# Zhiyu014/GNN-UDS

Hardware: AMD Instinct MI355X
Metric: graph-steps/sec (forward rollout), |V|=10k |E|=12k d=64 (higher is better)
Workload: dtype f32 storage/accumulate, GEMM operands as bf16 hi+lo split (3 MFMA products)

## Files before the change

### gnn_uds_amd/_lib.py

```python
import ctypes
import os

import numpy as np
import torch

_HERE = os.path.dirname(os.path.abspath(__file__))
LIB_PATH = os.environ.get('UDS_LIB_PATH') or os.path.join(_HERE, 'libuds_hip.so')

ABI_VERSION = 22
FLAG_EXACT_FP32, FLAG_REQUIRE_FUSED = 1, 2
PRECISION_FLAGS = {'bf16x3': 0, 'fp32': FLAG_EXACT_FP32}

ACT = {None: 0, 'linear': 0, 'relu': 1, 'tanh': 2, 'sigmoid': 3, 'hard_sigmoid': 4}

_c_i64 = ctypes.c_int64
_c_int = ctypes.c_int
_c_ptr = ctypes.c_void_p

SYMBOLS = {
    'uds_abi_version': (_c_int, []),
    'uds_last_error': (ctypes.c_char_p, []),
    'uds_csr_create': (_c_int, [_c_ptr, _c_ptr, _c_i64, _c_i64, _c_i64, ctypes.POINTER(_c_ptr)]),
    'uds_csr_destroy': (_c_int, [_c_ptr]),
    'uds_csr_shape': (_c_int, [_c_ptr, ctypes.POINTER(_c_i64), ctypes.POINTER(_c_i64), ctypes.POINTER(_c_i64),
                               ctypes.POINTER(ctypes.c_int32)]),
    'uds_csr_row_order': (_c_int, [_c_ptr, _c_ptr]),
    'uds_dense_act': (_c_int, [_c_ptr, _c_i64, _c_ptr, _c_i64, _c_i64, _c_ptr, _c_ptr, _c_i64, _c_int, _c_ptr, _c_ptr,
                               _c_ptr, _c_ptr, _c_ptr, _c_ptr]),
    'uds_csr_spmm': (_c_int, [_c_ptr, _c_ptr, _c_ptr, _c_i64, _c_i64, _c_ptr, _c_int, _c_ptr, _c_ptr]),
    'uds_conv1d_causal': (_c_int, [_c_ptr, _c_i64, _c_i64, _c_i64, _c_i64, _c_ptr, _c_ptr, _c_i64, _c_i64, _c_i64, _c_int, _c_ptr,
                                   _c_ptr]),
    'uds_dense_cumsum_heads': (_c_int, [_c_ptr, _c_i64, _c_i64, _c_i64, _c_ptr, _c_ptr, _c_ptr, _c_int, _c_ptr, _c_ptr, _c_ptr]),
    'uds_recurrent_fused': (_c_int, [_c_ptr, _c_i64, _c_ptr, _c_ptr, _c_ptr, _c_i64, _c_i64, _c_i64, _c_int, _c_ptr, _c_ptr]),
    'uds_recurrent_fused_supported': (_c_int, [_c_i64, _c_int]),
    'uds_recurrent_forward': (_c_int, [_c_ptr, _c_ptr, _c_ptr, _c_i64, _c_i64, _c_i64, _c_i64, _c_int, _c_ptr, _c_ptr]),
    'uds_attn_sum_pool': (_c_int, [_c_ptr, _c_ptr, _c_i64, _c_i64, _c_i64, _c_ptr, _c_ptr]),
    'uds_dropout': (_c_int, [_c_ptr, _c_i64, ctypes.c_float, ctypes.c_uint64, ctypes.c_uint64, _c_ptr, _c_ptr]),
    'uds_recurrent_forward_train': (_c_int, [_c_ptr, _c_ptr, _c_ptr, _c_i64, _c_i64, _c_i64, _c_i64, _c_int, _c_ptr, _c_ptr, _c_ptr]),
    'uds_recurrent_backward': (_c_int, [_c_ptr, _c_ptr, _c_ptr, _c_ptr, _c_ptr, _c_ptr, _c_i64, _c_i64, _c_i64, _c_int, _c_ptr, _c_ptr, _c_ptr]),
    'uds_recurrent_bwd_packed_bytes': (_c_i64, [_c_i64, _c_int]),
    'uds_recurrent_pack_bwd': (_c_int, [_c_ptr, _c_i64, _c_int, _c_ptr, _c_ptr]),
    'uds_recurrent_backward_h': (_c_int, [_c_ptr, _c_ptr, _c_ptr, _c_ptr, _c_ptr, _c_ptr, _c_i64, _c_i64, _c_i64, _c_i64, _c_int, _c_ptr, _c_ptr,
                                          _c_ptr]),
    'uds_rowgemm_packed_bytes': (_c_i64, [_c_i64, _c_i64]),
    'uds_rowgemm_pack': (_c_int, [_c_ptr, _c_i64, _c_i64, _c_ptr, _c_ptr]),
    'uds_gat_aggregate_masked': (_c_int, [_c_ptr, _c_ptr, _c_ptr, _c_ptr, _c_ptr, _c_ptr, _c_i64, _c_i64, _c_int, _c_ptr, _c_ptr]),
    'uds_gat_aggregate_coef': (_c_int, [_c_ptr, _c_ptr, _c_ptr, _c_ptr, _c_ptr, _c_ptr, _c_i64, _c_i64, _c_int, _c_ptr, _c_ptr]),
    'uds_diffusion_forward': (_c_int, [_c_ptr, _c_ptr, _c_ptr, _c_ptr, _c_ptr, _c_i64, _c_i64, _c_int, _c_ptr, _c_ptr]),
    'uds_diffusion_backward_workspace_floats': (_c_i64, [_c_i64, _c_i64, _c_i64, _c_i64]),
    'uds_diffusion_backward': (_c_int, [_c_ptr, _c_ptr, _c_ptr, _c_ptr, _c_ptr, _c_ptr, _c_ptr, _c_ptr, _c_ptr, _c_ptr, _c_i64, _c_i64,
                                        _c_i64, _c_int, _c_ptr, _c_ptr, _c_ptr, _c_ptr]),
    'uds_halo_pack': (_c_int, [_c_ptr, _c_i64, _c_ptr, _c_i64, _c_i64, _c_i64, _c_ptr, _c_i64, _c_ptr, _c_i64, _c_ptr, _c_ptr]),
    'uds_halo_unpack': (_c_int, [_c_ptr, _c_i64, _c_i64, _c_ptr, _c_i64, _c_ptr, _c_i64, _c_ptr, _c_i64, _c_ptr, _c_i64, _c_ptr]),
    'uds_halo_pack_all': (_c_int, [_c_ptr, _c_i64, _c_ptr, _c_i64, _c_i64, _c_i64, _c_ptr, _c_i64, _c_ptr, _c_i64, _c_ptr, _c_ptr, _c_i64,
                                   _c_ptr, _c_ptr]),
    'uds_halo_unpack_all': (_c_int, [_c_ptr, _c_i64, _c_i64, _c_ptr, _c_i64, _c_ptr, _c_i64, _c_ptr, _c_ptr, _c_i64, _c_ptr, _c_i64, _c_ptr,
                                     _c_i64, _c_ptr]),
    'uds_halo_pack_clear_all': (_c_int, [_c_ptr, _c_i64, _c_ptr, _c_i64, _c_i64, _c_i64, _c_ptr, _c_i64, _c_ptr, _c_i64, _c_ptr, _c_ptr,
                                         _c_i64, _c_ptr, _c_ptr]),
    'uds_halo_accumulate_all': (_c_int, [_c_ptr, _c_i64, _c_i64, _c_ptr, _c_ptr, _c_i64, _c_ptr, _c_i64, _c_ptr, _c_i64, _c_ptr, _c_ptr,
                                         _c_i64, _c_ptr, _c_i64, _c_ptr, _c_i64, _c_ptr]),
    'uds_remainder_packed_bytes': (_c_i64, [_c_i64, _c_i64]),
    'uds_remainder_pack': (_c_int, [_c_ptr, _c_i64, _c_i64, _c_ptr, _c_ptr]),
    'uds_remainder_workspace_bytes': (_c_i64, [_c_i64, _c_i64, _c_i64, _c_i64]),
    'uds_remainder_forward_dense': (_c_int, [_c_ptr, _c_i64, _c_i64, _c_ptr, _c_i64, _c_ptr, _c_ptr, _c_int, _c_i64, _c_i64, _c_ptr, _c_ptr, _c_ptr]),
    'uds_remainder_forward': (_c_int, [_c_ptr, _c_i64, _c_i64, _c_ptr, _c_i64, _c_i64, _c_ptr, _c_ptr, _c_ptr]),
    'uds_rowgemm_forward': (_c_int, [_c_ptr, _c_i64, _c_i64, _c_i64, _c_i64, _c_ptr, _c_ptr, _c_i64, _c_i64, _c_i64, _c_int, _c_ptr, _c_ptr]),
    'uds_rowgemm_forward_pair': (_c_int, [_c_ptr, _c_i64, _c_ptr, _c_ptr, _c_ptr, _c_ptr, _c_i64, _c_ptr, _c_ptr, _c_ptr, _c_i64, _c_i64, _c_i64, _c_i64,
                                          _c_i64, _c_i64, _c_int, _c_ptr]),
    'uds_rowgemm_forward_cat': (_c_int, [_c_ptr, _c_i64, _c_ptr, _c_i64, _c_i64, _c_i64, _c_i64, _c_ptr, _c_ptr, _c_i64, _c_i64, _c_i64, _c_int,
                                         _c_ptr, _c_i64, _c_i64, _c_ptr]),
    'uds_dense_cumsum': (_c_int, [_c_ptr, _c_i64, _c_i64, _c_i64, _c_ptr, _c_ptr, _c_ptr, _c_int, _c_ptr, _c_ptr]),
    'uds_cumsum_act': (_c_int, [_c_ptr, _c_ptr, _c_i64, _c_i64, _c_i64, _c_i64, _c_int, _c_ptr, _c_ptr]),
    'uds_flow_balance': (_c_int, [_c_ptr, _c_ptr, _c_ptr, _c_i64, _c_ptr, _c_ptr, _c_ptr, _c_ptr, _c_ptr]),
    'uds_gat_workspace_floats': (_c_i64, [_c_i64, _c_i64, _c_i64]),
    'uds_gat_forward': (_c_int, [_c_ptr, _c_ptr, _c_i64, _c_ptr, _c_i64, _c_i64, _c_ptr, _c_ptr, _c_ptr, _c_ptr, _c_i64,
                                 _c_int, _c_ptr, _c_ptr, _c_ptr]),
    'uds_gat_aggregate': (_c_int, [_c_ptr, _c_ptr, _c_ptr, _c_ptr, _c_ptr, _c_i64, _c_i64, _c_int, _c_ptr, _c_ptr]),
    'uds_gat_backward': (_c_int, [_c_ptr, _c_ptr, _c_ptr, _c_ptr, _c_ptr, _c_ptr, _c_ptr, _c_ptr, _c_ptr, _c_i64, _c_i64, _c_ptr,
                                  _c_ptr, _c_ptr, _c_ptr, _c_ptr, _c_ptr]),
    'uds_gat_backward_coef': (_c_int, [_c_ptr, _c_ptr, _c_ptr, _c_ptr, _c_ptr, _c_ptr, _c_ptr, _c_ptr, _c_ptr, _c_ptr, _c_i64, _c_i64, _c_ptr,
                                       _c_ptr, _c_ptr, _c_ptr, _c_ptr, _c_ptr]),
    'uds_gat_aggregate_ex': (_c_int, [_c_ptr, _c_ptr, _c_ptr, _c_ptr, _c_ptr, _c_ptr, _c_ptr, _c_i64, _c_i64, _c_int, _c_ptr, _c_ptr]),
    'uds_gat_backward_ex': (_c_int, [_c_ptr, _c_ptr, _c_ptr, _c_ptr, _c_ptr, _c_ptr, _c_ptr, _c_ptr, _c_ptr, _c_ptr, _c_ptr, _c_i64, _c_i64,
                                     _c_ptr, _c_ptr, _c_ptr, _c_ptr, _c_ptr, _c_ptr]),
    'uds_csr_sddmm': (_c_int, [_c_ptr, _c_ptr, _c_ptr, _c_i64, _c_i64, _c_ptr, _c_ptr]),
    'uds_wgrad_workspace_floats': (_c_i64, [_c_i64, _c_i64, _c_i64, _c_int]),
    'uds_wgrad': (_c_int, [_c_ptr, _c_ptr, _c_i64, _c_i64, _c_i64, _c_i64, _c_i64, _c_i64, _c_int, _c_ptr, _c_ptr, _c_ptr, _c_ptr]),
    'uds_network_create': (_c_int, [_c_ptr, _c_ptr, _c_ptr, _c_ptr, ctypes.POINTER(_c_ptr)]),
    'uds_network_destroy': (_c_int, [_c_ptr]),
    'uds_network_prepare': (_c_int, [_c_ptr, _c_i64, _c_i64]),
    'uds_network_plan_info': (_c_int, [_c_ptr, _c_ptr]),
    'uds_tile_plan_create': (_c_int, [_c_ptr] * 8 + [_c_i64, _c_i64] + [ctypes.c_int32] * 4 + [ctypes.POINTER(_c_ptr)]),
    'uds_tile_plan_destroy': (_c_int, [_c_ptr]),
    'uds_tile_plan_sizes': (_c_int, [_c_ptr, ctypes.POINTER(_c_i64), ctypes.POINTER(_c_i64), _c_ptr]),
    'uds_tile_plan_copy': (_c_int, [_c_ptr, _c_ptr, _c_ptr]),
    'uds_tile_plan_blocks': (_c_int, [_c_ptr, _c_ptr, ctypes.POINTER(_c_i64)]),
    'uds_roll_update': (_c_int, [_c_ptr] * 7 + [_c_i64, _c_ptr, _c_i64, _c_ptr, _c_i64, _c_i64, _c_i64, _c_int, _c_ptr, _c_ptr, _c_ptr, _c_ptr]),
    'uds_spatial_workspace_floats': (_c_i64, [_c_ptr, _c_i64, _c_i64, _c_i64]),
    'uds_spatial_packed_bytes': (_c_i64, []),
    'uds_spatial_pack_weights': (_c_int, [_c_ptr, _c_i64, _c_i64, _c_i64, _c_i64, _c_ptr, _c_ptr]),
    'uds_spatial_layer_forward': (_c_int, [_c_ptr, _c_ptr, _c_ptr, _c_i64, _c_ptr, _c_i64, _c_i64, _c_i64, _c_i64, _c_int,
                                           _c_int, _c_ptr, _c_ptr, _c_ptr, _c_ptr]),
    'uds_spatial_layer_forward_rem': (_c_int, [_c_ptr, _c_ptr, _c_ptr, _c_i64, _c_ptr, _c_i64, _c_ptr, _c_ptr, _c_i64, _c_i64, _c_i64, _c_int, _c_int,
                                      _c_ptr, _c_ptr, _c_ptr, _c_ptr]),
    'uds_spatial_layer_forward_split': (_c_int, [_c_ptr, _c_ptr, _c_ptr, _c_i64, _c_ptr, _c_i64, _c_ptr, _c_i64, _c_ptr, _c_i64, _c_i64,
                                                 _c_i64, _c_i64, _c_int, _c_int, _c_ptr, _c_ptr, _c_ptr, _c_ptr]),
}


class SpatialParams(ctypes.Structure):
    _fields_ = [(n, _c_ptr) for n in ('xe_k', 'xe_b', 'ex_k', 'ex_b', 'ne_n_val', 'ne_e_val',
                                      'gx_k', 'gx_as', 'gx_an', 'gx_b', 'ge_k', 'ge_as', 'ge_an', 'ge_b', 'packed')]


class UdsError(RuntimeError):
    pass


_lib = None


def load():
    global _lib
    if _lib is not None:
        return _lib
    if not os.path.exists(LIB_PATH):
        raise ImportError('%s is missing: the HIP engine is not built (run `python -m gnn_uds_amd.build`); '
                          'gnn_uds_amd has no CPU fallback' % LIB_PATH)
    lib = ctypes.CDLL(LIB_PATH)
    for name, (res, args) in SYMBOLS.items():
        fn = getattr(lib, name)
        fn.restype = res
        fn.argtypes = args
    if lib.uds_abi_version() != ABI_VERSION:
        raise ImportError('libuds_hip.so ABI %d, binding expects %d' % (lib.uds_abi_version(), ABI_VERSION))
    _lib = lib
    return lib


def _check(rc, what):
    if rc != 0:
        msg = load().uds_last_error()
        raise UdsError('%s failed (%d): %s' % (what, rc, msg.decode() if msg else '?'))


def _dev(t, name, allow_none=False):
    if t is None:
        if allow_none:
            return None
        raise UdsError('%s is required' % name)
    if not isinstance(t, torch.Tensor):
        raise UdsError('%s must be a torch.Tensor, got %r' % (name, type(t)))
    if not t.is_cuda:
        raise UdsError('%s is on %s: gnn_uds_amd runs on the MI355X only and has no CPU fallback' % (name, t.device))
    if t.dtype != torch.float32:
        raise UdsError('%s must be float32, got %s' % (name, t.dtype))
    if not t.is_contiguous():
        raise UdsError('%s must be contiguous' % name)
    _same_device(t.device.index, name)
    return t.data_ptr()


def _current_device():
    if not torch.cuda.is_available():
        raise UdsError('no HIP device is visible: gnn_uds_amd runs on the MI355X only and has no CPU fallback')
    return torch.cuda.current_device()


def _same_device(index, what):
    cur = _current_device()
    if index is not None and index != cur:
        raise UdsError('%s lives on cuda:%d but the current device is cuda:%d: call torch.cuda.set_device(%d) (one process per GPU) '
                       'or wrap the call in `with torch.cuda.device(%d):`' % (what, index, cur, index, index))


def _dev_i32(t, name):
    if not isinstance(t, torch.Tensor) or not t.is_cuda or t.dtype != torch.int32 or not t.is_contiguous():
        raise UdsError('%s must be a contiguous int32 HIP tensor' % name)
    _same_device(t.device.index, name)
    return t.data_ptr()


def _stream():
    return torch.cuda.current_stream().cuda_stream


def _out(out, shape, like, name):
    if out is None:
        return torch.empty(shape, device=like.device, dtype=torch.float32)
    if tuple(out.shape) != tuple(shape) or out.device != like.device:
        raise UdsError('%s must be %r on %s, got %r on %s' % (name, tuple(shape), like.device, tuple(out.shape), out.device))
    _dev(out, name)
    return out


# ... 16 lines not shown
        if self._t is None:
            rows = np.repeat(np.arange(self.n_rows, dtype=np.int64), np.diff(self._rowptr.astype(np.int64)))
            cols = self._col.astype(np.int64)
            order = np.lexsort((rows, cols))
            t_rowptr = np.zeros(self.n_cols + 1, dtype=np.int64)
            np.add.at(t_rowptr, cols + 1, 1)
            t_rowptr = np.cumsum(t_rowptr)

            class _T:
                pass
            t = _T()
            t.n_rows, t.n_cols, t.nnz = self.n_cols, self.n_rows, self.nnz
            t.rowptr, t.col = t_rowptr.astype(np.int32), rows[order].astype(np.int32)
            self._t = (CsrHandle(t), order.astype(np.int32))
        h, perm = self._t
        if not isinstance(perm, torch.Tensor) or perm.device != torch.device(device):
            perm = torch.as_tensor(np.asarray(perm.cpu() if isinstance(perm, torch.Tensor) else perm), dtype=torch.int32,
                                   device=device)
            self._t = (h, perm)
        return h, perm

    @property
    def ptr(self):
        _same_device(self.device, 'this CSR handle')
        return self._h

    def row_order(self):
        out = np.empty(self.n_rows, dtype=np.int32)
        _check(load().uds_csr_row_order(self._h, out.ctypes.data), 'uds_csr_row_order')
        return out

    def max_degree(self):
        md = ctypes.c_int32()
        _check(load().uds_csr_shape(self._h, None, None, None, ctypes.byref(md)), 'uds_csr_shape')
        return md.value

    def __del__(self):
        h, self._h = getattr(self, '_h', None), None
        if h is not None and _lib is not None:
            _lib.uds_csr_destroy(h)


class NetworkHandle:

    def __init__(self, graph):
        lib = load()
        self.graph = graph
        self.adj = CsrHandle(graph.adj)
        self.edge_adj = CsrHandle(graph.edge_adj)
        self.inc_n = CsrHandle(graph.inc_n)
        self.inc_e = CsrHandle(graph.inc_e)
        h = _c_ptr()
        self.device = _current_device()
        _check(lib.uds_network_create(self.adj.ptr, self.edge_adj.ptr, self.inc_n.ptr, self.inc_e.ptr, ctypes.byref(h)),
               'uds_network_create')
        self._h = h
        self._prepared = {(64, 64)}

    @property
    def ptr(self):
        _same_device(self.device, 'this network handle')
        return self._h

    def prepare(self, fx, fe):
        key = (int(fx), int(fe))
        if key not in self._prepared:
            _check(load().uds_network_prepare(self.ptr, key[0], key[1]), 'uds_network_prepare')
            self._prepared.add(key)

    def plan_info(self):
        info = np.zeros(8, dtype=np.int32)
        _check(load().uds_network_plan_info(self._h, info.ctypes.data), 'uds_network_plan_info')
        keys = ('fused', 'node_tiles', 'link_tiles', 'p_cap', 'q_cap', 'meta_cap', 'lds_bytes', 't_code')
        out = dict(zip(keys, (int(v) for v in info)))
        out['t_node'], out['t_link'] = out['t_code'] // 1000, out['t_code'] % 1000
        return out

    def __del__(self):
        h, self._h = getattr(self, '_h', None), None
        if h is not None and _lib is not None:
            _lib.uds_network_destroy(h)


def tile_plan(graph, t_node=48, t_link=48, p_limit=0, q_limit=0, blocks=False):
    lib = load()
    arrs = []
    for c in (graph.adj, graph.edge_adj, graph.inc_n, graph.inc_e):
        arrs += [np.ascontiguousarray(c.rowptr, dtype=np.int32), np.ascontiguousarray(c.col, dtype=np.int32)]
    h = _c_ptr()
    _check(lib.uds_tile_plan_create(*[a.ctypes.data for a in arrs], graph.n_node, graph.n_edge, t_node, t_link,
                                    p_limit, q_limit, ctypes.byref(h)), 'uds_tile_plan_create')
    try:
        nt, pl = _c_i64(), _c_i64()
        caps = np.zeros(3, dtype=np.int32)
        _check(lib.uds_tile_plan_sizes(h, ctypes.byref(nt), ctypes.byref(pl), caps.ctypes.data), 'uds_tile_plan_sizes')
        hdr = np.zeros((nt.value, 8), dtype=np.int32)
        pool = np.zeros(pl.value, dtype=np.int32)
        _check(lib.uds_tile_plan_copy(h, hdr.ctypes.data, pool.ctypes.data), 'uds_tile_plan_copy')
        blk = None
        if blocks:
            stride = _c_i64()
            if lib.uds_tile_plan_blocks(h, None, ctypes.byref(stride)) == 0:
                blk = np.zeros((nt.value, stride.value), dtype=np.int32)
                _check(lib.uds_tile_plan_blocks(h, blk.ctypes.data, ctypes.byref(stride)), 'uds_tile_plan_blocks')
    finally:
        lib.uds_tile_plan_destroy(h)
    out = dict(p_cap=int(caps[0]), q_cap=int(caps[1]), meta_cap=int(caps[2]))
    if blocks:
        out['blocks'] = blk
    return hdr, pool, out


def dense_act(xa, kernel, bias=None, act='linear', xb=None, attn=None):
    lib = load()
    fa = xa.shape[-1]
    fb = 0 if xb is None else xb.shape[-1]
    rows = xa.numel() // fa
    fo = kernel.shape[-1]
    if kernel.shape[0] != fa + fb:
        raise UdsError('kernel has %d input features, inputs give %d' % (kernel.shape[0], fa + fb))
    if xb is not None and xb.shape[:-1] != xa.shape[:-1]:
        raise UdsError('xa %r and xb %r disagree on leading dims' % (tuple(xa.shape), tuple(xb.shape)))
    out = torch.empty(xa.shape[:-1] + (fo,), device=xa.device, dtype=torch.float32)
    s_self = s_nbr = None
    if attn is not None:
        s_self = torch.empty(xa.shape[:-1], device=xa.device, dtype=torch.float32)
        s_nbr = torch.empty_like(s_self)
    if rows == 0:
        _dev(xa, 'xa')
        return (out, s_self, s_nbr) if attn is not None else out
    _check(lib.uds_dense_act(_dev(xa, 'xa'), fa, _dev(xb, 'xb', True), fb, rows, _dev(kernel, 'kernel'),
                             _dev(bias, 'bias', True), fo, ACT[act],
                             _dev(attn[0], 'a_self') if attn else None, _dev(attn[1], 'a_nbr') if attn else None,
                             _dev(out, 'out'), _dev(s_self, 's_self', True), _dev(s_nbr, 's_nbr', True), _stream()),
           'uds_dense_act')
    return (out, s_self, s_nbr) if attn is not None else out


def conv1d_causal(x, kernel, bias=None, dilation=1, act='linear'):
    lib = load()
    if x.dim() != 4 or kernel.dim() != 3 or kernel.shape[1] != x.shape[-1]:
        raise UdsError('conv1d_causal: x %r / kernel %r' % (tuple(x.shape), tuple(kernel.shape)))
    B, T, R, F = x.shape
    taps, _, H = kernel.shape
    out = torch.empty((B, T, R, H), device=x.device, dtype=torch.float32)
    if out.numel() == 0:
        _dev(x, 'x')
        return out
    _check(lib.uds_conv1d_causal(_dev(x, 'x'), B, T, R, F, _dev(kernel, 'kernel'), _dev(bias, 'bias', True), taps, dilation, H,
                                 ACT[act], _dev(out, 'out'), _stream()), 'uds_conv1d_causal')
    return out


def recurrent_fused_supported(F, kind):
    return bool(load().uds_recurrent_fused_supported(int(F), 0 if kind == 'GRU' else 1))


def recurrent_pack(kernel, recurrent_kernel):
    G = recurrent_kernel.shape[1] // 64
    if tuple(recurrent_kernel.shape) != (64, G * 64) or G not in (3, 4) or (kernel is not None and kernel.shape[1] != G * 64):
        raise UdsError('recurrent_pack: kernel %r / recurrent kernel %r (F x G*64 and 64 x G*64 with G = 3 or 4)'
                       % (None if kernel is None else tuple(kernel.shape), tuple(recurrent_kernel.shape)))
    mats = [recurrent_kernel] if kernel is None else [kernel, recurrent_kernel]
    return torch.cat([rowgemm_pack(m[:, 64 * g:64 * (g + 1)].contiguous()) for m in mats for g in range(G)]).contiguous()


def recurrent_fused(x, packed, b_in, b_rec, kind, projected=False):
    lib = load()
    B, T, R, F = x.shape
    out = torch.empty((B, T, R, 64), device=x.device, dtype=torch.float32)
    if out.numel():
        _check(lib.uds_recurrent_fused(_dev(x, 'x'), 0 if projected else F, packed.data_ptr(), _dev(b_in, 'b_in', True), _dev(b_rec, 'b_rec', True),
                                       B, T, R, 0 if kind == 'GRU' else 1, _dev(out, 'out'), _stream()), 'uds_recurrent_fused')
    return out


def attn_sum_pool(x, attn_kernel):
    lib = load()
    B, R, F = x.shape
    k = attn_kernel.reshape(-1).contiguous()
    if k.numel() != F:
        raise UdsError('attn_sum_pool: x %r, attn_kernel %r' % (tuple(x.shape), tuple(attn_kernel.shape)))
    out = torch.empty((B, F), device=x.device, dtype=torch.float32)
    if B:
        _check(lib.uds_attn_sum_pool(_dev(x, 'x'), _dev(k, 'attn_kernel'), B, R, F, _dev(out, 'out'), _stream()), 'uds_attn_sum_pool')
    return out


def dropout(x, rate, seed, offset):
    lib = load()
    x = x.contiguous()
    out = torch.empty_like(x)
# ... 518 lines not shown
        raise UdsError('%s %r for %d snapshots of a %d-entry pattern' % (name, tuple(t.shape), S, handle.nnz))


def gat_aggregate_ex(handle, hx, s_self, s_nbr, bias=None, act='relu', edge_mask=None, coef=None):
    lib = load()
    S, n, d = hx.shape
    if n != handle.n_rows or tuple(s_self.shape) != (S, n) or tuple(s_nbr.shape) != (S, n):
        raise UdsError('gat_aggregate_ex: hx %r, s_self %r, s_nbr %r do not match a %d-row pattern' %
                       (tuple(hx.shape), tuple(s_self.shape), tuple(s_nbr.shape), handle.n_rows))
    _check_entry_operand('gat_aggregate_ex: edge_mask', edge_mask, S, handle)
    _check_entry_operand('gat_aggregate_ex: coef', coef, S, handle)
    out = torch.empty_like(hx)
    if out.numel() == 0:
        _dev(hx, 'hx')
        return out
    _check(lib.uds_gat_aggregate_ex(handle.ptr, _dev(hx, 'hx'), _dev(s_self, 's_self'), _dev(s_nbr, 's_nbr'), _dev(bias, 'bias', True),
                                    _dev(edge_mask, 'edge_mask', True), _dev(coef, 'coef', True), S, d, ACT[act], _dev(out, 'out'),
                                    _stream()), 'uds_gat_aggregate_ex')
    return out


def gat_backward_ex(handle, handle_t, perm_t, grad, hx, s_self, s_nbr, a_self, a_nbr, edge_mask=None, coef=None):
    lib = load()
    S, n, d = grad.shape
    if n != handle.n_rows or tuple(hx.shape) != (S, n, d) or tuple(s_self.shape) != (S, n) or tuple(s_nbr.shape) != (S, n):
        raise UdsError('gat_backward_ex: grad %r, hx %r, s_self %r, s_nbr %r do not match a %d-row pattern' %
                       (tuple(grad.shape), tuple(hx.shape), tuple(s_self.shape), tuple(s_nbr.shape), handle.n_rows))
    _check_entry_operand('gat_backward_ex: edge_mask', edge_mask, S, handle)
    _check_entry_operand('gat_backward_ex: coef', coef, S, handle)
    d_hx = torch.empty_like(grad)
    ds_self = torch.empty((S, n), device=grad.device, dtype=torch.float32)
    ds_nbr = torch.empty_like(ds_self)
    if grad.numel() == 0:
        _dev(grad, 'grad')
        return d_hx, ds_self, ds_nbr
    ws = torch.empty((2, S, max(handle.nnz, 1)), device=grad.device, dtype=torch.float32)
    _check(lib.uds_gat_backward_ex(handle.ptr, handle_t.ptr, _dev_i32(perm_t, 'perm_t'), _dev(grad, 'grad'), _dev(hx, 'hx'),
                                   _dev(s_self, 's_self'), _dev(s_nbr, 's_nbr'), _dev(a_self, 'a_self'), _dev(a_nbr, 'a_nbr'),
                                   _dev(edge_mask, 'edge_mask', True), _dev(coef, 'coef', True), S, d, _dev(ws[0], 'alpha_ws'),
                                   _dev(ws[1], 'de_ws'), _dev(d_hx, 'd_hx'), _dev(ds_self, 'ds_self'), _dev(ds_nbr, 'ds_nbr'),
                                   _stream()), 'uds_gat_backward_ex')
    return d_hx, ds_self, ds_nbr


def wgrad_supported(F, H, with_bias=True):
    return load().uds_wgrad_workspace_floats(128, F, H, int(with_bias)) > 0


def wgrad(a, g, shift=0, with_bias=True):
    lib = load()
    B, T, R, F = a.shape
    H = g.shape[-1]
    if tuple(g.shape[:-1]) != (B, T, R):
        raise UdsError('wgrad: a %r and g %r disagree' % (tuple(a.shape), tuple(g.shape)))
    n_ws = lib.uds_wgrad_workspace_floats(max(B * T * R, 1), F, H, int(with_bias))
    if n_ws <= 0:
        raise UdsError('wgrad: F=%d / H=%d not supported' % (F, H))
    dk = torch.empty((F, H), device=a.device, dtype=torch.float32)
    db = torch.empty(H, device=a.device, dtype=torch.float32) if with_bias else None
    ws = torch.empty(n_ws, device=a.device, dtype=torch.float32)
    _check(lib.uds_wgrad(_dev(a, 'a'), _dev(g, 'g'), B, T, R, F, H, shift, int(with_bias), _dev(ws, 'workspace'), _dev(dk, 'd_kernel'),
                         _dev(db, 'd_bias', True), _stream()), 'uds_wgrad')
    return dk, db


def csr_sddmm(handle, a, b):
    lib = load()
    if a.dim() != 3 or b.dim() != 3 or a.shape[1] != handle.n_rows or b.shape[1] != handle.n_cols or a.shape[0] != b.shape[0] \
            or a.shape[2] != b.shape[2]:
        raise UdsError('sddmm: a must be (S,%d,F) and b (S,%d,F), got %r, %r' % (handle.n_rows, handle.n_cols, tuple(a.shape),
                                                                               tuple(b.shape)))
    out = torch.zeros(handle.nnz, device=a.device, dtype=torch.float32)
    if handle.nnz == 0 or a.numel() == 0:
        _dev(a, 'a')
        return out
    _check(lib.uds_csr_sddmm(handle.ptr, _dev(a, 'a'), _dev(b, 'b'), a.shape[0], a.shape[2], _dev(out, 'out'), _stream()),
           'uds_csr_sddmm')
    return out


def _spatial_params(p):
    sp = SpatialParams()
    for name, _ in SpatialParams._fields_:
        if name == 'packed':
            t = p.get('packed')
            sp.packed = None if t is None else t.data_ptr()
        else:
            setattr(sp, name, _dev(p[name], name, allow_none=name.endswith('_b')))
    return sp


def spatial_pack_weights(p, fx, fe, h, d):
    lib = load()
    out = torch.empty(lib.uds_spatial_packed_bytes() // 4, device=p['xe_k'].device, dtype=torch.float32)
    q = dict(p)
    q['packed'] = None
    _check(lib.uds_spatial_pack_weights(ctypes.byref(_spatial_params(q)), fx, fe, h, d, out.data_ptr(), _stream()),
           'uds_spatial_pack_weights')
    return out


def spatial_layer_forward(net, p, x, e, h, d, act='relu', flags=0, xb=None, eb=None, rem_x=None, rem_e=None):
    lib = load()
    S, N, fx = x.shape
    _, E, fe = e.shape
    if e.shape[0] != S or N != net.graph.n_node or E != net.graph.n_edge:
        raise UdsError('x %r / e %r do not match the network (N=%d, E=%d)' % (tuple(x.shape), tuple(e.shape),
                                                                            net.graph.n_node, net.graph.n_edge))
    if S == 0:
        _dev(x, 'x')
        return (torch.empty((0, N, d), device=x.device, dtype=torch.float32),
                torch.empty((0, E, d), device=x.device, dtype=torch.float32))
    sp = _spatial_params(p)
    ws = torch.empty(lib.uds_spatial_workspace_floats(net.ptr, S, h, d), device=x.device, dtype=torch.float32)
    out_x = torch.empty((S, N, d), device=x.device, dtype=torch.float32)
    out_e = torch.empty((S, E, d), device=x.device, dtype=torch.float32)
    if rem_x is not None or rem_e is not None:
        if xb is not None or eb is not None or rem_x is None or rem_e is None:
            raise UdsError('rem_x and rem_e come together, without xb / eb')
        if tuple(rem_x.shape) != (S, N, h) or tuple(rem_e.shape) != (S, E, h):
            raise UdsError('rem_x %r / rem_e %r must be %r / %r' % (tuple(rem_x.shape), tuple(rem_e.shape), (S, N, h), (S, E, h)))
        _check(lib.uds_spatial_layer_forward_rem(net.ptr, ctypes.byref(sp), _dev(x, 'x'), fx, _dev(e, 'e'), fe, _dev(rem_x, 'rem_x'),
                                                 _dev(rem_e, 'rem_e'), S, h, d, ACT[act], int(flags), _dev(ws, 'workspace'),
                                                 _dev(out_x, 'out_x'), _dev(out_e, 'out_e'), _stream()), 'uds_spatial_layer_forward_rem')
        return out_x, out_e
    if xb is not None or eb is not None:
        for t, ref, name in ((xb, x, 'xb'), (eb, e, 'eb')):
            if t is not None and tuple(t.shape[:2]) != tuple(ref.shape[:2]):
                raise UdsError('%s %r does not match %r' % (name, tuple(t.shape), tuple(ref.shape)))
        _check(lib.uds_spatial_layer_forward_split(net.ptr, ctypes.byref(sp), _dev(x, 'x'), fx, _dev(xb, 'xb', True),
                                                   0 if xb is None else xb.shape[-1], _dev(e, 'e'), fe, _dev(eb, 'eb', True),
                                                   0 if eb is None else eb.shape[-1], S, h, d, ACT[act], int(flags),
                                                   _dev(ws, 'workspace'), _dev(out_x, 'out_x'), _dev(out_e, 'out_e'), _stream()),
               'uds_spatial_layer_forward_split')
        return out_x, out_e
    _check(lib.uds_spatial_layer_forward(net.ptr, ctypes.byref(sp), _dev(x, 'x'), fx, _dev(e, 'e'), fe, S, h, d, ACT[act],
                                         int(flags), _dev(ws, 'workspace'), _dev(out_x, 'out_x'), _dev(out_e, 'out_e'), _stream()),
           'uds_spatial_layer_forward')
    return out_x, out_e
```

### gnn_uds_amd/csrc/kernels_fused.hpp

```cpp
#pragma once
#include <hip/hip_runtime.h>
#include <stdint.h>

#include <type_traits>

#include "kernels_dense.hpp"
#include "kernels_sparse.hpp"
#include "tile_plan.hpp"

namespace uds {

typedef __attribute__((ext_vector_type(8))) __bf16 bf16x8;
typedef __attribute__((ext_vector_type(4))) float f32x4;

constexpr int FUSED_H = 32;
constexpr int FUSED_D = 64;
constexpr int FUSED_WAVES = 8;
constexpr int FUSED_U = 4;
constexpr int SEC_STRIDE = FUSED_H + 4;

struct FusedSide {
  const float *prim_in, *sec_in;
  const float *prim_in2, *sec_in2;
  float *out;
  const uint4 *w_small, *w_big;
  const uint4 *w_big32, *w_small32;
  const float *b_small, *a_self, *a_nbr, *b_out, *ne_val;
  int n_prim_glob, n_sec_glob;
  const float *rem;
};

struct FusedArgs {
  FusedSide side[2];
  const int32_t *hdr, *pool;
  const int32_t *blocks;
  int n_tiles, S, chunk, p_cap, q_cap, meta_cap, act, side_mask;
  unsigned long long *dbg;
};

__device__ __forceinline__ int frag_k(int t, int qd, int jj) { return 32 * t + (jj < 4 ? 4 * qd + jj : 16 + 4 * qd + (jj - 4)); }

__global__ void k_pack_weight_frags(const float *__restrict__ W, int K, int F_out, uint4 *__restrict__ out) {
  const int MB = F_out / 16, KT = K / 32;
  const int idx = blockIdx.x * blockDim.x + threadIdx.x;
  if (idx >= KT * MB * 64) return;
  const int lane = idx & 63, m = (idx >> 6) % MB, t = (idx >> 6) / MB;
  const int qd = lane >> 4, f = 16 * m + (lane & 15);
  bf16x8 hi, lo;
#pragma unroll
  for (int jj = 0; jj < 8; ++jj) {
    const float w = W[(int64_t)frag_k(t, qd, jj) * F_out + f];
    const __bf16 h = (__bf16)w;
    hi[jj] = h;
    lo[jj] = (__bf16)(w - (float)h);
  }
  out[((t * MB + m) * 2 + 0) * 64 + lane] = __builtin_bit_cast(uint4, hi);
  out[((t * MB + m) * 2 + 1) * 64 + lane] = __builtin_bit_cast(uint4, lo);
}

__global__ void k_pack_weight_frags32(const float *__restrict__ W, int K, int F_out, uint4 *__restrict__ out) {
  const int MB = F_out / 32, KT = K / 16;
  const int idx = blockIdx.x * blockDim.x + threadIdx.x;
  if (idx >= KT * MB * 64) return;
  const int lane = idx & 63, m = (idx >> 6) % MB, t = (idx >> 6) / MB;
  const int hf = lane >> 5, f = 32 * m + (lane & 31);
  bf16x8 hi, lo;
#pragma unroll
  for (int jj = 0; jj < 8; ++jj) {
    const float w = W[(int64_t)(16 * t + 8 * hf + jj) * F_out + f];
    const __bf16 h = (__bf16)w;
    hi[jj] = h;
    lo[jj] = (__bf16)(w - (float)h);
  }
  out[((t * MB + m) * 2 + 0) * 64 + lane] = __builtin_bit_cast(uint4, hi);
  out[((t * MB + m) * 2 + 1) * 64 + lane] = __builtin_bit_cast(uint4, lo);
}

__device__ __forceinline__ void split8(const float4 &a, const float4 &b, bf16x8 &hi, bf16x8 &lo) {
  typedef float f32x2_t __attribute__((ext_vector_type(2)));
  typedef __bf16 bf16x2_t __attribute__((ext_vector_type(2)));
  const f32x2_t v[4] = {{a.x, a.y}, {a.z, a.w}, {b.x, b.y}, {b.z, b.w}};
  unsigned hw[4], lw[4];
#pragma unroll
  for (int p = 0; p < 4; ++p) {
    const bf16x2_t h = __builtin_convertvector(v[p], bf16x2_t);
    const unsigned hb = __builtin_bit_cast(unsigned, h);
    const f32x2_t hf = {__uint_as_float(hb << 16), __uint_as_float(hb & 0xffff0000u)};
    const bf16x2_t l = __builtin_convertvector(v[p] - hf, bf16x2_t);
    hw[p] = hb;
    lw[p] = __builtin_bit_cast(unsigned, l);
  }
  hi = __builtin_bit_cast(bf16x8, make_uint4(hw[0], hw[1], hw[2], hw[3]));
  lo = __builtin_bit_cast(bf16x8, make_uint4(lw[0], lw[1], lw[2], lw[3]));
}

__device__ __forceinline__ f32x4 mfma3(const bf16x8 &wh, const bf16x8 &wl, const bf16x8 &dh, const bf16x8 &dl, f32x4 acc) {
  acc = __builtin_amdgcn_mfma_f32_16x16x32_bf16(wh, dl, acc, 0, 0, 0);
  acc = __builtin_amdgcn_mfma_f32_16x16x32_bf16(wl, dh, acc, 0, 0, 0);
  acc = __builtin_amdgcn_mfma_f32_16x16x32_bf16(wh, dh, acc, 0, 0, 0);
  return acc;
}

template <int CTRL>
__device__ __forceinline__ float row_dpp(float v) {
  const int x = __builtin_bit_cast(int, v);
  return __builtin_bit_cast(float, __builtin_amdgcn_update_dpp(x, x, CTRL, 0xf, 0xf, true));
}
__device__ __forceinline__ float row16_max(float v) {
  v = fmaxf(v, row_dpp<0xB1>(v));
  v = fmaxf(v, row_dpp<0x4E>(v));
  v = fmaxf(v, row_dpp<0x124>(v));
  v = fmaxf(v, row_dpp<0x128>(v));
  return v;
// ... 145 lines not shown
                 : "=&s"(keep)
                 : "v"(voff), "s"(base), "s"(lds_byte)
                 : "memory", "scc");
  } else {
    asm volatile("s_mov_b32 %0, m0\n\ts_mov_b32 m0, %3\n\ts_nop 4\n\tglobal_load_lds_dwordx4 %1, %2\n\t"
                 "s_add_u32 m0, m0, 0x3c0\n\ts_nop 0\n\tglobal_load_lds_dwordx4 %1, %2 offset:64\n\t"
                 "s_add_u32 m0, m0, 0x3c0\n\ts_nop 0\n\tglobal_load_lds_dwordx4 %1, %2 offset:128\n\t"
                 "s_add_u32 m0, m0, 0x3c0\n\ts_nop 0\n\tglobal_load_lds_dwordx4 %1, %2 offset:192\n\t"
                 "s_add_u32 m0, m0, 0x3c0\n\ts_nop 0\n\tglobal_load_lds_dwordx4 %1, %2 offset:256\n\t"
                 "s_add_u32 m0, m0, 0x3c0\n\ts_nop 0\n\tglobal_load_lds_dwordx4 %1, %2 offset:320\n\ts_mov_b32 m0, %0"
                 : "=&s"(keep)
                 : "v"(voff), "s"(base), "s"(lds_byte)
                 : "memory", "scc");
  }
}
__device__ __forceinline__ unsigned lds_addr(const void *p) {
  return (unsigned)(uintptr_t)(const __attribute__((address_space(3))) void *)p;
}

template <int FP, int FS, int ACT>
__global__ __launch_bounds__(FUSED_WAVES * 64, 2) void k_fused_tile(FusedArgs a) {
  constexpr int NW = FUSED_WAVES, NT = FUSED_WAVES * 64;
  constexpr int KT_S = FS / 32, MB_S = FUSED_H / 16;
  constexpr int KT_X = FP / 32, KT_B = KT_X + 1, MB_B = FUSED_D / 16;
  constexpr int U = FUSED_U;
  extern __shared__ __attribute__((aligned(16))) int32_t smem[];
#ifdef UDS_PHASE_TIMING
  unsigned long long tm_[12] = {0, 0, 0, 0, 0, 0, 0, 0, 0, 0, 0, 0}, tl_ = clock64();
  const unsigned long long rt0_ = __builtin_amdgcn_s_memrealtime(), mt0_ = tl_;
#define UDS_STAMP(k) do { const unsigned long long n_ = clock64(); tm_[k] += n_ - tl_; tl_ = n_; } while (0)
#else
#define UDS_STAMP(k) do { } while (0)
#endif

  const int tid = threadIdx.x, lane = tid & 63;
  const int wave = __builtin_amdgcn_readfirstlane(tid >> 6);
  const int r16 = lane & 15, qd = lane >> 4;
  const int c16 = r16, rs = qd;
#ifdef UDS_PRIO_YOUNG
  if (wave >= 4) __builtin_amdgcn_s_setprio(1);
#endif

  const int W = gridDim.x, b = blockIdx.x;
  const int q8 = W / 8, r8 = W % 8, xcd = b % 8;
  const int w = (xcd < r8 ? xcd * (q8 + 1) : r8 * (q8 + 1) + (xcd - r8) * q8) + b / 8;
  const int tile = w % a.n_tiles;
  const int chunk_id = w / a.n_tiles;
  const int s_begin = chunk_id * a.chunk;
  const int s_end = min(a.S, (chunk_id + 1) * a.chunk);
  const int sd = __builtin_amdgcn_readfirstlane(a.hdr[tile * TILE_HDR_INTS + 6]);
  if (!((a.side_mask >> sd) & 1)) return;
  const FusedSide &S_ = a.side[sd];
  constexpr bool COLD_X = FP > 64, COLD_S = FS > 64 || SMALL_IN_LDS;
  constexpr int T_COLD_X = KT_X - 1, T_COLD_S = SMALL_IN_LDS ? 0 : KT_S - 1;
  constexpr int N_COLD_S = (KT_S - T_COLD_S) * MB_S * 2 * 64;
  float *s_self = reinterpret_cast<float *>(smem + a.meta_cap);
  float *s_nbr = s_self + a.p_cap;
  float *attn = s_nbr + a.p_cap;
  uint4 *cold_b = reinterpret_cast<uint4 *>(attn + 2 * FUSED_D + FUSED_H);
  uint4 *cold_s = cold_b + (COLD_X ? MB_B * 2 * 64 : 0);
  bf16x8 wsh[KT_S][MB_S], wsl[KT_S][MB_S], wbh[KT_B][MB_B], wbl[KT_B][MB_B];
#pragma unroll
  for (int t = 0; t < KT_S; ++t)
#pragma unroll
    for (int m = 0; m < MB_S; ++m) {
      if (COLD_S && t >= T_COLD_S) continue;
      wsh[t][m] = __builtin_bit_cast(bf16x8, S_.w_small[((t * MB_S + m) * 2 + 0) * 64 + lane]);
      wsl[t][m] = __builtin_bit_cast(bf16x8, S_.w_small[((t * MB_S + m) * 2 + 1) * 64 + lane]);
    }
#pragma unroll
  for (int t = 0; t < KT_B; ++t)
#pragma unroll
    for (int m = 0; m < MB_B; ++m) {
      if (COLD_X && t == T_COLD_X) continue;
      wbh[t][m] = __builtin_bit_cast(bf16x8, S_.w_big[((t * MB_B + m) * 2 + 0) * 64 + lane]);
      wbl[t][m] = __builtin_bit_cast(bf16x8, S_.w_big[((t * MB_B + m) * 2 + 1) * 64 + lane]);
    }
  if (COLD_X)
    for (int i = tid; i < MB_B * 2 * 64; i += NT) cold_b[i] = S_.w_big[T_COLD_X * MB_B * 2 * 64 + i];
  if (COLD_S)
    for (int i = tid; i < N_COLD_S; i += NT) cold_s[i] = S_.w_small[T_COLD_S * MB_S * 2 * 64 + i];
  f32x4 bo = f32x4{0.f, 0.f, 0.f, 0.f};
  if (S_.b_out) bo = *reinterpret_cast<const f32x4 *>(S_.b_out + 4 * c16);
  {
    const uint4 *src = reinterpret_cast<const uint4 *>(a.blocks + (int64_t)tile * a.meta_cap);
    uint4 *dst = reinterpret_cast<uint4 *>(smem);
    for (int i = tid; i < a.meta_cap / 4; i += NT) dst[i] = src[i];
  }
  if (tid < FUSED_D) {
    attn[tid] = S_.a_self[tid] * 1.44269504088896340736f;
    attn[FUSED_D + tid] = S_.a_nbr[tid] * 1.44269504088896340736f;
    if (tid < FUSED_H) attn[2 * FUSED_D + tid] = S_.b_small ? S_.b_small[tid] : 0.f;
  }
  __syncthreads();
  UDS_STAMP(7);
  const int n_own = __builtin_amdgcn_readfirstlane(smem[0]), n_prim = __builtin_amdgcn_readfirstlane(smem[1]),
            n_sec = __builtin_amdgcn_readfirstlane(smem[2]), flags = __builtin_amdgcn_readfirstlane(smem[3]),
            n_ovf = __builtin_amdgcn_readfirstlane(smem[4]), n_adj = __builtin_amdgcn_readfirstlane(smem[5]),
            inc_width = __builtin_amdgcn_readfirstlane(smem[7]);
  const EllOffsets off = ell_offsets(n_own, n_prim, n_sec, flags, n_ovf, n_adj);

  float *sec = reinterpret_cast<float *>(cold_s + (COLD_S ? N_COLD_S : 0));
  float *hx = sec + a.q_cap * SEC_STRIDE;
  float *stage_s = hx + a.p_cap * FUSED_D;
  float *stage_p = stage_s + a.q_cap * FS;

  const int32_t *prim_ids = smem + off.prim;
  const int32_t *sec_ids = smem + off.sec;
  const uint32_t *inc_loc = reinterpret_cast<const uint32_t *>(smem + off.inc_loc);
  int32_t *inc_w = smem + off.inc_w;
  const f32x4 *inc_val4 = reinterpret_cast<const f32x4 *>(inc_w);
  const unsigned char *adj_b = reinterpret_cast<const unsigned char *>(smem + off.adj);
  const int32_t *ovf_ptr = smem + off.ovf_ptr, *ovf_loc = smem + off.ovf_loc;
  int32_t *ovf_w = smem + off.ovf_w;
  const int32_t *adj_ptr = smem + off.adj_ptr, *adj_loc = smem + off.adj_loc;
  auto sec_row = [&](int blk) { return sec_ids[min(blk * 16 + r16, n_sec - 1)]; };
  auto prim_row = [&](int blk) { return prim_ids[min(blk * 16 + r16, n_prim - 1)]; };
  const int srow0 = wave * 16 < n_sec ? sec_row(wave) : 0, srow1 = (wave + NW) * 16 < n_sec ? sec_row(wave + NW) : 0;
  const int prow0 = wave * 16 < n_prim ? prim_row(wave) : 0;
  const bool sec_split = FS == 96 && S_.sec_in2 != nullptr, prim_split = FP == 96 && S_.prim_in2 != nullptr;
  const int64_t sec_stride = (int64_t)S_.n_sec_glob * (sec_split ? 64 : FS), sec_stride2 = (int64_t)S_.n_sec_glob * 32;
  const int64_t prim_stride = (int64_t)S_.n_prim_glob * (prim_split ? 64 : FP), prim_stride2 = (int64_t)S_.n_prim_glob * 32;
  const float *sec_next = S_.sec_in + s_begin * sec_stride, *sec_next2 = sec_split ? S_.sec_in2 + s_begin * sec_stride2 : nullptr;
  const float *prim_next = S_.prim_in + s_begin * prim_stride, *prim_next2 = prim_split ? S_.prim_in2 + s_begin * prim_stride2 : nullptr;
  auto dma_sec = [&](int blk) {
    const unsigned row = (unsigned)(blk == wave ? srow0 : (blk == wave + NW ? srow1 : sec_row(blk)));
    const unsigned dst = __builtin_amdgcn_readfirstlane(lds_addr(stage_s) + (unsigned)blk * (KT_S * 2 * 1024));
    if (sec_split) {
      glds16_run_s<4>(sec_next, row * 256u + 16u * qd, dst);
      glds16_run_s<2>(sec_next2, row * 128u + 16u * qd, dst + 4096u);
    } else {
      glds16_run_s<2 * KT_S>(sec_next, row * (unsigned)(FS * 4) + 16u * qd, dst);
    }
  };
  auto dma_prim = [&](int blk) {
    const unsigned row = (unsigned)(blk == wave ? prow0 : prim_row(blk));
    const unsigned dst = __builtin_amdgcn_readfirstlane(lds_addr(stage_p) + (unsigned)blk * (KT_X * 2 * 1024));
    if (prim_split) {
      glds16_run_s<4>(prim_next, row * 256u + 16u * qd, dst);
      glds16_run_s<2>(prim_next2, row * 128u + 16u * qd, dst + 4096u);
    } else {
      glds16_run_s<2 * KT_X>(prim_next, row * (unsigned)(FP * 4) + 16u * qd, dst);
    }
  };
  auto sec_advance = [&]() { sec_next += sec_stride; if (sec_split) sec_next2 += sec_stride2; };
  auto prim_advance = [&]() { prim_next += prim_stride; if (prim_split) prim_next2 += prim_stride2; };

  int p3_dmax[U];
#pragma unroll
  for (int u = 0; u < U; ++u) {
    const int i = wave * 4 + 4 * NW * u + rs;
    const int ic = min(i, n_own - 1);
    int dmx;
    if (flags & ELL_FLAG_LONG_ROWS) {
      dmx = i < n_own ? adj_ptr[ic + 1] - adj_ptr[ic] : 0;
    } else {
      const unsigned long long m = __ballot(i < n_own && adj_b[ic * ELL_ADJ + c16] != 0xFF);
      dmx = __builtin_popcountll((m >> (16 * rs)) & 0xffffull);
    }
    dmx = max(dmx, __shfl_xor(dmx, 16));
    dmx = max(dmx, __shfl_xor(dmx, 32));
    p3_dmax[u] = __builtin_amdgcn_readfirstlane(dmx);
  }

  const int np_sec = sec_split ? 6 : 2 * KT_S, np_prim = prim_split ? 6 : 2 * KT_X;
  int vm_since_sec = 0, vm_since_prim = 0;
  if (s_begin < s_end) {
    for (int blk = wave; blk * 16 < n_sec; blk += NW) dma_sec(blk);
    for (int blk = wave; blk * 16 < n_prim; blk += NW) {
      dma_prim(blk);
      vm_since_sec += np_prim;
    }
    sec_advance();
    prim_advance();
  }
#ifdef UDS_PHASE_TIMING
  const unsigned long long t_dma_issued_ = clock64();
#endif
  for (int i = tid; i < ELL_INC * n_prim; i += NT) {
    const int k = inc_w[i];
    reinterpret_cast<float *>(inc_w)[i] = k >= 0 ? S_.ne_val[k] : 0.f;
  }
  if (flags & ELL_FLAG_INC_OVF)
    for (int i = tid; i < n_ovf; i += NT) reinterpret_cast<float *>(ovf_w)[i] = S_.ne_val[ovf_w[i]];
  const float *ovf_val = reinterpret_cast<const float *>(ovf_w);
#ifdef UDS_PHASE_TIMING
  const unsigned long long t_loads_issued_ = clock64();
#endif
  __syncthreads();
  UDS_STAMP(0);

  auto phase1 = [&](int s) {
    if (wave * 16 < n_sec) wait_vm(vm_since_sec);
    UDS_STAMP(1);
    const bool more = s + 1 < s_end;
    for (int blk = wave; blk * 16 < n_sec; blk += NW) {
      const float4 *st = reinterpret_cast<const float4 *>(stage_s + blk * (KT_S * 2 * 256)) + lane;
      bf16x8 dh[KT_S], dl[KT_S];
#pragma unroll
      for (int t = 0; t < KT_S; ++t) split8(st[(2 * t) * 64], st[(2 * t + 1) * 64], dh[t], dl[t]);
      const int lrow = blk * 16 + r16;
      f32x4 acc[MB_S];
#pragma unroll
      for (int m = 0; m < MB_S; ++m) acc[m] = *reinterpret_cast<const f32x4 *>(attn + 2 * FUSED_D + 16 * m + 4 * qd);
#pragma unroll
      for (int t = 0; t < KT_S; ++t)
#pragma unroll
        for (int m = 0; m < MB_S; ++m) {
          if (COLD_S && t >= T_COLD_S)
            acc[m] = mfma3(__builtin_bit_cast(bf16x8, cold_s[(((t - T_COLD_S) * MB_S + m) * 2 + 0) * 64 + lane]),
                           __builtin_bit_cast(bf16x8, cold_s[(((t - T_COLD_S) * MB_S + m) * 2 + 1) * 64 + lane]), dh[t], dl[t], acc[m]);
          else
            acc[m] = mfma3(wsh[t][m], wsl[t][m], dh[t], dl[t], acc[m]);
        }
      if (more) {
        __builtin_amdgcn_sched_barrier(0);
        asm volatile("s_waitcnt lgkmcnt(0)" ::: "memory");
        dma_sec(blk);
        vm_since_prim += np_sec;
        vm_since_sec = 0;
        __builtin_amdgcn_sched_barrier(0);
      }
      if (lrow < n_sec) {
#pragma unroll
        for (int m = 0; m < MB_S; ++m) {
          f32x4 o;
#pragma unroll
          for (int j = 0; j < 4; ++j) o[j] = fused_act<ACT>(acc[m][j], a.act);
          *reinterpret_cast<f32x4 *>(sec + lrow * SEC_STRIDE + 16 * m + 4 * qd) = o;
        }
      }
    }
    if (more) sec_advance();
    UDS_STAMP(2);
  };

  unsigned p3_jb[U];
  auto phase2 = [&](int s, unsigned ag_locs, f32x4 ag_vals) {
    if (wave * 16 < n_prim) wait_vm(vm_since_prim);
    const bool more = s + 1 < s_end;
    for (int blk = wave; blk * 16 < n_prim; blk += NW) {
      const float4 *st = reinterpret_cast<const float4 *>(stage_p + blk * (KT_X * 2 * 256)) + lane;
      bf16x8 dh[KT_B], dl[KT_B];
#pragma unroll
      for (int t = 0; t < KT_X; ++t) split8(st[(2 * t) * 64], st[(2 * t + 1) * 64], dh[t], dl[t]);
      UDS_STAMP(8);
      const int lrow = blk * 16 + r16;
      const bool valid = lrow < n_prim;
      const int lr = min(lrow, n_prim - 1);
      f32x4 acc[MB_B];
#pragma unroll
      for (int m = 0; m < MB_B; ++m) acc[m] = f32x4{0.f, 0.f, 0.f, 0.f};
#pragma unroll
      for (int t = 0; t < KT_X; ++t)
#pragma unroll
        for (int m = 0; m < MB_B; ++m) {
          if (COLD_X && t == T_COLD_X)
            acc[m] = mfma3(__builtin_bit_cast(bf16x8, cold_b[(m * 2 + 0) * 64 + lane]), __builtin_bit_cast(bf16x8, cold_b[(m * 2 + 1) * 64 + lane]),
                           dh[t], dl[t], acc[m]);
          else
            acc[m] = mfma3(wbh[t][m], wbl[t][m], dh[t], dl[t], acc[m]);
        }
      unsigned locs = ag_locs;
      f32x4 vals = ag_vals;
      if (blk != wave) {
        locs = inc_loc[lr];
        vals = inc_val4[lr];
      }
      if (more) {
        __builtin_amdgcn_sched_barrier(0);
        asm volatile("s_waitcnt lgkmcnt(0)" ::: "memory");
        dma_prim(blk);
// ... 223 lines not shown
```

### gnn_uds_amd/csrc/kernels_fused_ws.hpp

```cpp
#pragma once
#include "kernels_fused.hpp"

namespace uds {

#ifndef UDS_WS_NY
#define UDS_WS_NY 4
#endif
#ifndef UDS_WS_SLOTS
#define UDS_WS_SLOTS 4
#endif
constexpr int WS_NY = UDS_WS_NY, WS_NX = FUSED_WAVES - WS_NY;
#ifdef UDS_WS_YG
constexpr int WS_YG = UDS_WS_NY;
#else
constexpr int WS_YG = 0;
#endif
constexpr int WS_SLOTS = UDS_WS_SLOTS;
#ifndef UDS_WS_PRE
#define UDS_WS_PRE 0
#endif
constexpr int WS_PRE = UDS_WS_PRE;
static_assert(WS_PRE % WS_SLOTS == 0, "WS_PRE must be a multiple of WS_SLOTS");
#ifndef UDS_WS_XPRIO
#define UDS_WS_XPRIO 1
// ... 6 lines not shown

template <int IMM>
__device__ __forceinline__ void ws_gld16(f32x4 &dst, const float *base, unsigned voff) {
  asm volatile("global_load_dwordx4 %0, %1, %2 offset:%3" : "=v"(dst) : "v"(voff), "s"(base), "n"(IMM) : "memory");
}
__device__ __forceinline__ void ws_pin4(f32x4 &a0, f32x4 &a1, f32x4 &a2, f32x4 &a3) {
  asm volatile("" : "+v"(a0), "+v"(a1), "+v"(a2), "+v"(a3));
}
__device__ __forceinline__ void row8_max4(const float (&in)[4], float (&out)[4]) {
  asm("s_nop 1\n\t" UDS_DPP4_FIRST("v_max_f32_dpp", "quad_perm:[1,0,3,2]") UDS_DPP4("v_max_f32_dpp", "quad_perm:[2,3,0,1]")
      UDS_DPP4("v_max_f32_dpp", "row_half_mirror")
      : "=&v"(out[0]), "=&v"(out[1]), "=&v"(out[2]), "=&v"(out[3])
      : "v"(in[0]), "v"(in[1]), "v"(in[2]), "v"(in[3]));
}
__device__ __forceinline__ void row8_sum4(const float (&in)[4], float (&out)[4]) {
  asm("s_nop 1\n\t" UDS_DPP4_FIRST("v_add_f32_dpp", "quad_perm:[1,0,3,2]") UDS_DPP4("v_add_f32_dpp", "quad_perm:[2,3,0,1]")
      UDS_DPP4("v_add_f32_dpp", "row_half_mirror")
      : "=&v"(out[0]), "=&v"(out[1]), "=&v"(out[2]), "=&v"(out[3])
      : "v"(in[0]), "v"(in[1]), "v"(in[2]), "v"(in[3]));
}
template <int HI>
__device__ __forceinline__ unsigned ws_add_half(unsigned pk, unsigned base) {
  unsigned r;
  if (HI) asm("v_add_u32_sdwa %0, %1, %2 dst_sel:DWORD dst_unused:UNUSED_PAD src0_sel:WORD_1 src1_sel:DWORD" : "=v"(r) : "v"(pk), "v"(base));
  else asm("v_add_u32_sdwa %0, %1, %2 dst_sel:DWORD dst_unused:UNUSED_PAD src0_sel:WORD_0 src1_sel:DWORD" : "=v"(r) : "v"(pk), "v"(base));
  return r;
}
__device__ __forceinline__ void ws_vmcnt(int n) {
  switch (n) {
    case 0: asm volatile("s_waitcnt vmcnt(0)" ::: "memory"); break;
    case 1: asm volatile("s_waitcnt vmcnt(1)" ::: "memory"); break;
    case 2: asm volatile("s_waitcnt vmcnt(2)" ::: "memory"); break;
    case 3: asm volatile("s_waitcnt vmcnt(3)" ::: "memory"); break;
    case 4: asm volatile("s_waitcnt vmcnt(4)" ::: "memory"); break;
    case 5: asm volatile("s_waitcnt vmcnt(5)" ::: "memory"); break;
    case 6: asm volatile("s_waitcnt vmcnt(6)" ::: "memory"); break;
    case 7: asm volatile("s_waitcnt vmcnt(7)" ::: "memory"); break;
    default: asm volatile("s_waitcnt vmcnt(8)" ::: "memory"); break;
  }
}

template <int ACT>
__global__ __launch_bounds__(FUSED_WAVES * 64, 2) void k_fused_ws(FusedArgs a) {
  constexpr int NT = FUSED_WAVES * 64, NY = WS_NY, NX = WS_NX;
  constexpr int FP = 64, FS = 64;
  constexpr int KT_S = FS / 32, MB_S = FUSED_H / 16;
  constexpr int KT_X = FP / 32, KT_B = KT_X + 1, MB_B = FUSED_D / 16;
  constexpr int U = FUSED_U;
  constexpr int PJ = (8 + NY - 1) / NY;
  constexpr int SJ = (16 + NX - 1) / NX;
  extern __shared__ __attribute__((aligned(16))) int32_t smem[];

  const int tid = threadIdx.x, lane = tid & 63;
  const int wave = __builtin_amdgcn_readfirstlane(tid >> 6);
#ifdef UDS_WS_PAIR_SAME
  static_assert(NY == 4, "UDS_WS_PAIR_SAME assumes 4 + 4");
  const bool team_y = (wave & 3) < 2;
  const int yw = (wave & 1) + 2 * (wave >> 2), xw = ((wave & 3) - 2) + 2 * (wave >> 2);
#else
  const bool team_y = wave < NY;
  const int yw = wave, xw = wave - NY;
#endif
  const int r16 = lane & 15, qd = lane >> 4;
  const int c16 = r16, rs = qd;

  const int W = gridDim.x, b = blockIdx.x;
  const int q8 = W / 8, r8 = W % 8, xcd = b % 8;
  const int w = (xcd < r8 ? xcd * (q8 + 1) : r8 * (q8 + 1) + (xcd - r8) * q8) + b / 8;
  const int tile = w % a.n_tiles;
  const int chunk_id = w / a.n_tiles;
  const int s_begin = chunk_id * a.chunk;
  const int s_end = min(a.S, (chunk_id + 1) * a.chunk);
  const int sd = __builtin_amdgcn_readfirstlane(a.hdr[tile * TILE_HDR_INTS + 6]);
  if (!((a.side_mask >> sd) & 1)) return;
  const FusedSide &S_ = a.side[sd];

  float *s_self = reinterpret_cast<float *>(smem + a.meta_cap);
  float *s_nbr = s_self + 2 * a.p_cap;
  float *attn = s_nbr + 2 * a.p_cap;
  float *sec = attn + 3 * FUSED_D + FUSED_H;
  float *hx = sec + 2 * a.q_cap * SEC_STRIDE;
  const int sec_buf = a.q_cap * SEC_STRIDE, hx_buf = a.p_cap * FUSED_D;

  {
    const uint4 *src = reinterpret_cast<const uint4 *>(a.blocks + (int64_t)tile * a.meta_cap);
    uint4 *dst = reinterpret_cast<uint4 *>(smem);
    for (int i = tid; i < a.meta_cap / 4; i += NT) dst[i] = src[i];
  }
  if (tid < FUSED_D) {
    attn[tid] = S_.a_self[tid] * 1.44269504088896340736f;
    attn[FUSED_D + tid] = S_.a_nbr[tid] * 1.44269504088896340736f;
    if (tid < FUSED_H) attn[2 * FUSED_D + tid] = S_.b_small ? S_.b_small[tid] : 0.f;
    attn[2 * FUSED_D + FUSED_H + tid] = S_.b_out ? S_.b_out[tid] : 0.f;
  }
  __syncthreads();
  const int n_own = __builtin_amdgcn_readfirstlane(smem[0]), n_prim = __builtin_amdgcn_readfirstlane(smem[1]),
            n_sec = __builtin_amdgcn_readfirstlane(smem[2]), flags = __builtin_amdgcn_readfirstlane(smem[3]),
            n_ovf = __builtin_amdgcn_readfirstlane(smem[4]), n_adj = __builtin_amdgcn_readfirstlane(smem[5]),
            inc_width = __builtin_amdgcn_readfirstlane(smem[7]);
  const EllOffsets off = ell_offsets(n_own, n_prim, n_sec, flags, n_ovf, n_adj);
  const int32_t *prim_ids = smem + off.prim;
  const int32_t *sec_ids = smem + off.sec;
  const uint32_t *inc_loc = reinterpret_cast<const uint32_t *>(smem + off.inc_loc);
  int32_t *inc_w = smem + off.inc_w;
  const f32x4 *inc_val4 = reinterpret_cast<const f32x4 *>(inc_w);
  const unsigned char *adj_b = reinterpret_cast<const unsigned char *>(smem + off.adj);
  const int32_t *ovf_ptr = smem + off.ovf_ptr, *ovf_loc = smem + off.ovf_loc;
  int32_t *ovf_w = smem + off.ovf_w;
  const int32_t *adj_ptr = smem + off.adj_ptr, *adj_loc = smem + off.adj_loc;

  for (int i = tid; i < ELL_INC * n_prim; i += NT) {
    const int k = inc_w[i];
    reinterpret_cast<float *>(inc_w)[i] = k >= 0 ? S_.ne_val[k] : 0.f;
  }
  if (flags & ELL_FLAG_INC_OVF)
    for (int i = tid; i < n_ovf; i += NT) reinterpret_cast<float *>(ovf_w)[i] = S_.ne_val[ovf_w[i]];
  const float *ovf_val = reinterpret_cast<const float *>(ovf_w);

#ifdef UDS_PHASE_TIMING
  unsigned long long tm_[8] = {0, 0, 0, 0, 0, 0, 0, 0}, tl_ = clock64();
  const unsigned long long rt0_ = __builtin_amdgcn_s_memrealtime(), mt0_ = tl_;
#define WS_STAMP(k) do { const unsigned long long n_ = clock64(); tm_[k] += n_ - tl_; tl_ = n_; } while (0)
#define WS_DUMP() do { if (a.dbg && lane == 0) { unsigned long long *o = a.dbg + ((size_t)blockIdx.x * 8 + wave) * 16; \
    for (int q_ = 0; q_ < 7; ++q_) o[q_] = tm_[q_]; o[12] = wave; \
    o[15] = ((__builtin_amdgcn_s_memrealtime() - rt0_) << 32) | ((clock64() - mt0_) & 0xffffffffull); \
    o[7] = 1ull | ((unsigned long long)sd << 8) | ((unsigned long long)n_own << 16) | ((unsigned long long)n_prim << 32) | ((unsigned long long)n_sec << 48); } } while (0)
#else
#define WS_STAMP(k) do { } while (0)
#define WS_DUMP() do { } while (0)
#endif
  const int64_t sec_stride = (int64_t)S_.n_sec_glob * FS, prim_stride = (int64_t)S_.n_prim_glob * FP;
  const int n_snap = s_end - s_begin;

  __syncthreads();
  if (team_y) {
#ifndef UDS_WS_MFMA16
    typedef float f32x16 __attribute__((ext_vector_type(16)));
    constexpr int KT32 = (FP + FUSED_H) / 16, KX32 = FP / 16, MB32 = FUSED_D / 32;
    static_assert(NY == 4, "one 32-row block per Y wave: four waves cover p_cap = 128");
    const int n32 = lane & 31, hf = lane >> 5;
    bf16x8 wh[KT32][MB32], wl[KT32][MB32];
#pragma unroll
    for (int t = 0; t < KT32; ++t)
#pragma unroll
      for (int m = 0; m < MB32; ++m) {
        wh[t][m] = __builtin_bit_cast(bf16x8, S_.w_big32[((t * MB32 + m) * 2 + 0) * 64 + lane]);
        wl[t][m] = __builtin_bit_cast(bf16x8, S_.w_big32[((t * MB32 + m) * 2 + 1) * 64 + lane]);
      }
    const int lrow = 32 * yw + n32;
    const bool valid = lrow < n_prim;
    const int lr = min(lrow, n_prim - 1);
    const unsigned prow = (unsigned)prim_ids[lr] * FP + 8u * hf;
    f32x4 pp[2 * KX32];
    const bool has_rem = S_.rem != nullptr;
    const unsigned rrow = (unsigned)prim_ids[lr] * FUSED_H + 8u * hf;
    f32x4 rm[4] = {f32x4{0.f, 0.f, 0.f, 0.f}, f32x4{0.f, 0.f, 0.f, 0.f}, f32x4{0.f, 0.f, 0.f, 0.f}, f32x4{0.f, 0.f, 0.f, 0.f}};
    const int64_t rem_stride = (int64_t)S_.n_prim_glob * FUSED_H;
    const unsigned ag_locs = inc_loc[lr];
    const f32x4 ag_vals = inc_val4[lr];
    __builtin_amdgcn_s_waitcnt(0x0F70);
    if (n_snap > 0) {
      const float *base = S_.prim_in + s_begin * prim_stride;
      static_for<2 * KX32>([&](auto i_) {
        constexpr int i = decltype(i_)::value;
        pp[i] = *reinterpret_cast<const f32x4 *>(base + prow + 16 * (i >> 1) + 4 * (i & 1));
      });
      if (has_rem) {
        const float *rb = S_.rem + s_begin * rem_stride + rrow;
        rm[0] = *reinterpret_cast<const f32x4 *>(rb);
        rm[1] = *reinterpret_cast<const f32x4 *>(rb + 4);
        rm[2] = *reinterpret_cast<const f32x4 *>(rb + 16);
        rm[3] = *reinterpret_cast<const f32x4 *>(rb + 20);
      }
    }
    WS_STAMP(0);
    lds_barrier();

    auto mfma3_32 = [&](const bf16x8 &a_h, const bf16x8 &a_l, const bf16x8 &d_h, const bf16x8 &d_l, f32x16 acc) __attribute__((always_inline)) {
      acc = __builtin_amdgcn_mfma_f32_32x32x16_bf16(a_h, d_l, acc, 0, 0, 0);
      acc = __builtin_amdgcn_mfma_f32_32x32x16_bf16(a_l, d_h, acc, 0, 0, 0);
      acc = __builtin_amdgcn_mfma_f32_32x32x16_bf16(a_h, d_h, acc, 0, 0, 0);
      return acc;
    };
    for (int k = 0; k <= n_snap; ++k) {
#ifdef UDS_WS_ABL_NO_P2
      if (false) {
#else
      if (k < n_snap && 32 * yw < n_prim) {
#endif
        const bool more = k + 1 < n_snap;
        const float *next = S_.prim_in + (s_begin + k + 1) * prim_stride;
        const float *secr = sec + (k & 1) * sec_buf;
        float *hxw = hx + (k & 1) * hx_buf;
        float *ssw = s_self + (k & 1) * a.p_cap, *snw = s_nbr + (k & 1) * a.p_cap;
        bf16x8 dh[KT32], dl[KT32];
        static_for<KX32>([&](auto t_) {
          constexpr int t = decltype(t_)::value;
          const f32x4 u0 = pp[2 * t], u1 = pp[2 * t + 1];
          split8(make_float4(u0[0], u0[1], u0[2], u0[3]), make_float4(u1[0], u1[1], u1[2], u1[3]), dh[t], dl[t]);
        });
        if (more)
          static_for<2 * KX32>([&](auto i_) {
            constexpr int i = decltype(i_)::value;
            pp[i] = *reinterpret_cast<const f32x4 *>(next + prow + 16 * (i >> 1) + 4 * (i & 1));
          });
        f32x16 acc[MB32];
#pragma unroll
        for (int m = 0; m < MB32; ++m)
#pragma unroll
          for (int r = 0; r < 16; ++r) acc[m][r] = 0.f;
#pragma unroll
        for (int t = 0; t < KX32; ++t)
#pragma unroll
          for (int m = 0; m < MB32; ++m) acc[m] = mfma3_32(wh[t][m], wl[t][m], dh[t], dl[t], acc[m]);
        float4 g0 = make_float4(rm[0][0], rm[0][1], rm[0][2], rm[0][3]), g1 = make_float4(rm[1][0], rm[1][1], rm[1][2], rm[1][3]),
               g2 = make_float4(rm[2][0], rm[2][1], rm[2][2], rm[2][3]), g3 = make_float4(rm[3][0], rm[3][1], rm[3][2], rm[3][3]);
        if (more && has_rem) {
// ... 213 lines not shown
            for (int t = 0; t < KT_X; ++t)
#pragma unroll
              for (int m = 0; m < MB_B; ++m) acc[m] = mfma3(wbh[t][m], wbl[t][m], dh[t], dl[t], acc[m]);
#else
#pragma unroll
            for (int m = 0; m < MB_B; ++m) acc[m] = f32x4{__builtin_bit_cast(float, (unsigned)dh[0][0] << 16), (float)m, __builtin_bit_cast(float, (unsigned)dl[1][0] << 16), 0.f};
#endif
            const unsigned locs = ag_locs[j];
            const f32x4 vals = ag_vals[j];
            float4 g0 = make_float4(0.f, 0.f, 0.f, 0.f), g1 = g0;
            auto fma_row = [&](float wv, const float4 &u0, const float4 &u1) {
              g0.x = fmaf(wv, u0.x, g0.x); g0.y = fmaf(wv, u0.y, g0.y); g0.z = fmaf(wv, u0.z, g0.z); g0.w = fmaf(wv, u0.w, g0.w);
              g1.x = fmaf(wv, u1.x, g1.x); g1.y = fmaf(wv, u1.y, g1.y); g1.z = fmaf(wv, u1.z, g1.z); g1.w = fmaf(wv, u1.w, g1.w);
            };
            auto add2 = [&](unsigned la, float wa, unsigned lb, float wb) {
              const float *ra = secr + la * SEC_STRIDE + 4 * qd, *rb = secr + lb * SEC_STRIDE + 4 * qd;
              const float4 a0 = *reinterpret_cast<const float4 *>(ra), a1 = *reinterpret_cast<const float4 *>(ra + 16);
              const float4 b0 = *reinterpret_cast<const float4 *>(rb), b1 = *reinterpret_cast<const float4 *>(rb + 16);
              fma_row(wa, a0, a1);
              fma_row(wb, b0, b1);
            };
#ifndef UDS_WS_ABL_Y_NO_AGG
            add2(locs & 0xffu, vals[0], (locs >> 8) & 0xffu, vals[1]);
            if (inc_width > 2) add2((locs >> 16) & 0xffu, vals[2], locs >> 24, vals[3]);
#else
            g0.x = vals[0]; g1.y = vals[1]; g0.z = __uint_as_float(locs);
#endif
            if (flags & ELL_FLAG_INC_OVF)
              for (int p = ovf_ptr[lr]; p < ovf_ptr[lr + 1]; ++p) {
                const float *ra = secr + ovf_loc[p] * SEC_STRIDE + 4 * qd;
                fma_row(ovf_val[p], *reinterpret_cast<const float4 *>(ra), *reinterpret_cast<const float4 *>(ra + 16));
              }
            split8(g0, g1, dh[KT_X], dl[KT_X]);
#ifndef UDS_WS_ABL_Y_NO_MFMA
#pragma unroll
            for (int m = 0; m < MB_B; ++m) acc[m] = mfma3(wbh[KT_X][m], wbl[KT_X][m], dh[KT_X], dl[KT_X], acc[m]);
#else
            acc[0][3] += __builtin_bit_cast(float, (unsigned)dh[KT_X][0] << 16) + __builtin_bit_cast(float, (unsigned)dl[KT_X][0] << 16);
#endif
            typedef float f32x2 __attribute__((ext_vector_type(2)));
            f32x2 ps2 = {0.f, 0.f}, pn2 = {0.f, 0.f};
#pragma unroll
            for (int m = 0; m < MB_B; ++m) {
              const f32x4 as4 = *reinterpret_cast<const f32x4 *>(attn + 16 * m + 4 * qd);
              const f32x4 an4 = *reinterpret_cast<const f32x4 *>(attn + FUSED_D + 16 * m + 4 * qd);
              ps2 = __builtin_elementwise_fma(acc[m].xy, as4.xy, ps2);
              pn2 = __builtin_elementwise_fma(acc[m].xy, an4.xy, pn2);
              ps2 = __builtin_elementwise_fma(acc[m].zw, as4.zw, ps2);
              pn2 = __builtin_elementwise_fma(acc[m].zw, an4.zw, pn2);
            }
            const float ps = quarters_sum(ps2.x + ps2.y);
            const float pn = quarters_sum(pn2.x + pn2.y);
#ifdef UDS_WS_ABL_Y_NO_HXW
            if (valid && ps == 12345.f) {
#else
            if (valid) {
#endif
              if (qd == 0) {
                ssw[lrow] = ps;
                snw[lrow] = pn;
              }
#pragma unroll
              for (int m = 0; m < MB_B; ++m)
                *reinterpret_cast<f32x4 *>(hxw + lrow * FUSED_D + (((4 * m + qd) ^ (lrow & 7)) << 2)) = acc[m];
            }
          }
        });
      }
      if (WS_YG > 0 && k >= 1) phase3_y(s_begin + k - 1, (k - 1) & 1);
      WS_STAMP(1);
      lds_barrier();
      WS_STAMP(2);
    }
    WS_DUMP();
#endif
  } else {
#ifndef UDS_WS_NO_PRIO
    __builtin_amdgcn_s_setprio(UDS_WS_XPRIO);
#endif
#ifndef UDS_WS_MFMA16
    typedef float f32x16 __attribute__((ext_vector_type(16)));
    constexpr int KS32 = FS / 16, SJ32 = (8 + NX - 1) / NX;
    const int n32 = lane & 31, hf = lane >> 5;
    bf16x8 w1h[KS32], w1l[KS32];
#pragma unroll
    for (int t = 0; t < KS32; ++t) {
      w1h[t] = __builtin_bit_cast(bf16x8, S_.w_small32[(t * 2 + 0) * 64 + lane]);
      w1l[t] = __builtin_bit_cast(bf16x8, S_.w_small32[(t * 2 + 1) * 64 + lane]);
    }
    unsigned srow[SJ32];
#pragma unroll
    for (int j = 0; j < SJ32; ++j) srow[j] = ((unsigned)sec_ids[min((xw + NX * j) * 32 + n32, n_sec - 1)] * FS + 8u * hf) * 4u;
    f32x4 sp[SJ32][2 * KS32];
    auto load_sec_at = [&](const float *base) __attribute__((always_inline)) {
      static_for<SJ32>([&](auto j_) {
        constexpr int j = decltype(j_)::value;
        ws_gld16<0>(sp[j][0], base, srow[j]);
        ws_gld16<16>(sp[j][1], base, srow[j]);
        ws_gld16<64>(sp[j][2], base, srow[j]);
        ws_gld16<80>(sp[j][3], base, srow[j]);
        ws_gld16<128>(sp[j][4], base, srow[j]);
        ws_gld16<144>(sp[j][5], base, srow[j]);
        ws_gld16<192>(sp[j][6], base, srow[j]);
        ws_gld16<208>(sp[j][7], base, srow[j]);
      });
    };
    auto load_sec = [&](int s) __attribute__((always_inline)) { load_sec_at(S_.sec_in + s * sec_stride); };
#define UDS_WS_RUNNING_PTRS 1
#else
    bf16x8 wsh[KT_S][MB_S], wsl[KT_S][MB_S];
#pragma unroll
    for (int t = 0; t < KT_S; ++t)
#pragma unroll
      for (int m = 0; m < MB_S; ++m) {
        wsh[t][m] = __builtin_bit_cast(bf16x8, S_.w_small[((t * MB_S + m) * 2 + 0) * 64 + lane]);
        wsl[t][m] = __builtin_bit_cast(bf16x8, S_.w_small[((t * MB_S + m) * 2 + 1) * 64 + lane]);
      }
    unsigned srow[SJ];
#pragma unroll
    for (int j = 0; j < SJ; ++j) srow[j] = ((unsigned)sec_ids[min((xw + NX * j) * 16 + r16, n_sec - 1)] * FS + 4u * qd) * 4u;
    f32x4 sp[SJ][2 * KT_S];
    auto load_sec = [&](int s) __attribute__((always_inline)) {
      const float *base = S_.sec_in + s * sec_stride;
      static_for<SJ>([&](auto j_) {
        constexpr int j = decltype(j_)::value;
        ws_gld16<0>(sp[j][0], base, srow[j]);
        ws_gld16<64>(sp[j][1], base, srow[j]);
        ws_gld16<128>(sp[j][2], base, srow[j]);
        ws_gld16<192>(sp[j][3], base, srow[j]);
      });
    };
#endif
#ifndef UDS_WS_OCT_WD
#define UDS_WS_OCT_WD 4
#endif
#ifndef UDS_WS_OCT_GRP
#define UDS_WS_OCT_GRP 1
#endif
#ifndef UDS_WS_P3_GROUPS
    const int ro = lane >> 3, c8 = lane & 7, hf8 = ro & 1;
    int p3_dmax[U];
    unsigned p3_pk[U][4];
    unsigned p3_jb4 = 0;
    int n_st = 0;
#pragma unroll
    for (int u = 0; u < U; ++u) {
      const int i = 8 * (NX * u + xw) + ro;
      const int ic = min(i, n_own - 1);
      int dmx;
      if (flags & ELL_FLAG_LONG_ROWS) {
        dmx = i < n_own ? adj_ptr[ic + 1] - adj_ptr[ic] : 0;
      } else {
        const unsigned long long m0 = __ballot(i < n_own && adj_b[ic * ELL_ADJ + c8] != 0xFF);
        const unsigned long long m1 = __ballot(i < n_own && adj_b[ic * ELL_ADJ + 8 + c8] != 0xFF);
        dmx = __builtin_popcountll((m0 >> (8 * ro)) & 0xffull) + __builtin_popcountll((m1 >> (8 * ro)) & 0xffull);
      }
#pragma unroll
      for (int o = 8; o < 64; o <<= 1) dmx = max(dmx, __shfl_xor(dmx, o));
      p3_dmax[u] = __builtin_amdgcn_readfirstlane(dmx);
#pragma unroll
      for (int k2 = 0; k2 < 4; ++k2) {
        unsigned pk = 0;
#pragma unroll
        for (int h = 0; h < 2; ++h) {
          const unsigned jb = adj_b[ic * ELL_ADJ + 2 * k2 + h];
          const unsigned j = (i < n_own && jb != 0xFFu) ? jb : 0u;
          pk |= (j * (FUSED_D * 4) + (((j & 7) ^ c8) << 4)) << (16 * h);
        }
        p3_pk[u][k2] = pk;
      }
      p3_jb4 |= (i < n_own ? (unsigned)adj_b[i * ELL_ADJ + c8] : 0xFFu) << (8 * u);
// ... 524 lines not shown
```

### gnn_uds_amd/csrc/tile_plan.hpp

```cpp
#pragma once
#include <algorithm>
#include <cmath>
#include <cstdint>
#include <numeric>
#include <vector>

namespace uds {

struct HostCsr {
  int64_t n_rows = 0, n_cols = 0;
  std::vector<int32_t> rowptr, col;
};

constexpr int TILE_HDR_INTS = 8;
inline int tile_block_ints(int meta_cap) { return (TILE_HDR_INTS + meta_cap + 3) & ~3; }

struct SidePlan {
  int n_tiles = 0;
  int p_cap = 0, q_cap = 0, meta_cap = 0;
  std::vector<int32_t> hdr;
  std::vector<int32_t> pool;
  std::vector<int32_t> key;
  std::vector<int32_t> bfs_index;
};
// ... 325 lines not shown
  v.sec = v.prim + v.n_prim;
  v.inc_ptr = v.sec + v.n_sec;
  v.inc_loc = v.inc_ptr + v.n_prim + 1;
  v.inc_w = v.inc_loc + v.n_inc;
  v.adj_ptr = v.inc_w + v.n_inc;
  v.adj_loc = v.adj_ptr + v.n_own + 1;
  return v;
}
inline void ell_shape(const TileView &v, int &flags, int &n_ovf, int &inc_width) {
  flags = 0; n_ovf = 0; inc_width = 0;
  for (int i = 0; i < v.n_prim; ++i) {
    const int d = v.inc_ptr[i + 1] - v.inc_ptr[i];
    inc_width = std::max(inc_width, std::min(d, ELL_INC));
    if (d > ELL_INC) { flags |= ELL_FLAG_INC_OVF; n_ovf += d - ELL_INC; }
  }
  for (int i = 0; i < v.n_own; ++i)
    if (v.adj_ptr[i + 1] - v.adj_ptr[i] > ELL_ADJ) flags |= ELL_FLAG_LONG_ROWS;
}
inline bool ell_fits(const int32_t *hd) { return hd[1] <= 255 && hd[2] <= 256; }
inline int ell_block_len(const int32_t *hd, const int32_t *pool) {
  const TileView v = tile_view(hd, pool);
  int flags, n_ovf, w;
  ell_shape(v, flags, n_ovf, w);
  return ell_offsets(v.n_own, v.n_prim, v.n_sec, flags, n_ovf, v.n_adj).len;
}
inline int ell_block_cap(const std::vector<int32_t> &hdr, const std::vector<int32_t> &pool, int n_tiles) {
  int cap = 4;
  for (int t = 0; t < n_tiles; ++t) {
    const int32_t *hd = hdr.data() + (size_t)t * TILE_HDR_INTS;
    if (!ell_fits(hd)) return -1;
    cap = std::max(cap, ell_block_len(hd, pool.data()));
  }
  return cap;
}
inline void build_ell_blocks(const std::vector<int32_t> &hdr, const std::vector<int32_t> &pool, int n_tiles, int stride,
                             std::vector<int32_t> &out) {
  out.assign(std::max<size_t>((size_t)stride * n_tiles, 4), 0);
  for (int t = 0; t < n_tiles; ++t) {
    const int32_t *hd = hdr.data() + (size_t)t * TILE_HDR_INTS;
    const TileView v = tile_view(hd, pool.data());
    int flags, n_ovf, w;
    ell_shape(v, flags, n_ovf, w);
    const EllOffsets o = ell_offsets(v.n_own, v.n_prim, v.n_sec, flags, n_ovf, v.n_adj);
    int32_t *b = out.data() + (size_t)stride * t;
    const int32_t h[TILE_HDR_INTS] = {v.n_own, v.n_prim, v.n_sec, flags, n_ovf, (flags & ELL_FLAG_LONG_ROWS) ? v.n_adj : 0, v.side, w};
    std::copy(h, h + TILE_HDR_INTS, b);
    std::copy(v.prim, v.prim + v.n_prim, b + o.prim);
    std::copy(v.sec, v.sec + v.n_sec, b + o.sec);
    int q = 0;
    if (flags & ELL_FLAG_INC_OVF) b[o.ovf_ptr] = 0;
    for (int i = 0; i < v.n_prim; ++i) {
      uint32_t locs = 0;
      for (int k = 0; k < ELL_INC; ++k) {
        const int p = v.inc_ptr[i] + k;
        const bool has = p < v.inc_ptr[i + 1];
        if (has) locs |= (uint32_t)v.inc_loc[p] << (8 * k);
        b[o.inc_w + ELL_INC * i + k] = has ? v.inc_w[p] : -1;
      }
      b[o.inc_loc + i] = (int32_t)locs;
      if (flags & ELL_FLAG_INC_OVF) {
        for (int p = v.inc_ptr[i] + ELL_INC; p < v.inc_ptr[i + 1]; ++p, ++q) {
          b[o.ovf_loc + q] = v.inc_loc[p];
          b[o.ovf_w + q] = v.inc_w[p];
        }
        b[o.ovf_ptr + i + 1] = q;
      }
    }
    for (int i = 0; i < v.n_own; ++i)
      for (int c = 0; c < ELL_ADJ / 4; ++c) {
        uint32_t word = 0;
        for (int k = 0; k < 4; ++k) {
          const int p = v.adj_ptr[i] + 4 * c + k;
          word |= (uint32_t)(p < v.adj_ptr[i + 1] ? v.adj_loc[p] : 0xFF) << (8 * k);
        }
        b[o.adj + (ELL_ADJ / 4) * i + c] = (int32_t)word;
      }
    if (flags & ELL_FLAG_LONG_ROWS) {
      std::copy(v.adj_ptr, v.adj_ptr + v.n_own + 1, b + o.adj_ptr);
      std::copy(v.adj_loc, v.adj_loc + v.n_adj, b + o.adj_loc);
    }
  }
}

inline int64_t fused_lds_bytes(int p_cap, int q_cap, int meta_cap, int h, int d, int fp, int fs) {
  const int64_t weights = 16 * 64 * 2 * ((int64_t)(fs / 32) * (h / 16) + (int64_t)((fp + h) / 32) * (d / 16));
  const int64_t stage = std::max<int64_t>(4 * ((int64_t)q_cap * fs + (int64_t)p_cap * fp), weights);
#ifdef UDS_SMALL_IN_LDS
  const int64_t cold = (fp > 64 ? (d / 16) * 2 * 1024 : 0) + (int64_t)(fs / 32) * (h / 16) * 2 * 1024;
#else
  const int64_t cold = (fp > 64 ? (d / 16) * 2 * 1024 : 0) + (fs > 64 ? (h / 16) * 2 * 1024 : 0);
#endif
  return 4 * ((int64_t)meta_cap + 2 * p_cap + 2 * d + h + (int64_t)q_cap * (h + 4) + (int64_t)p_cap * d) + cold + stage;
}

struct NetworkPlan {
  SidePlan side[2];
  std::vector<int32_t> hdr;
  std::vector<int32_t> pool;
  int n_tiles = 0, p_cap = 0, q_cap = 0, meta_cap = 0, t_max[2] = {0, 0};
};

inline NetworkPlan build_network_plan(const HostCsr &adj, const HostCsr &eadj, const HostCsr &inc_n, const HostCsr &inc_e,
                                      int t_node, int t_link, int p_limit = 0, int q_limit = 0) {
  NetworkPlan np;
  np.t_max[0] = t_node;
  np.t_max[1] = t_link;
  np.side[0] = build_side_plan(adj, inc_n, t_node, 0, nullptr, p_limit, q_limit);
  np.side[1] = build_side_plan(eadj, inc_e, t_link, 1, &np.side[0].bfs_index, p_limit, q_limit);
  struct Ref { int32_t key, side, idx; };
  std::vector<Ref> refs;
  for (int s = 0; s < 2; ++s)
    for (int t = 0; t < np.side[s].n_tiles; ++t) refs.push_back({np.side[s].key[t], s, t});
  std::stable_sort(refs.begin(), refs.end(), [](const Ref &a, const Ref &b) { return a.key < b.key; });
  const int32_t base1 = (int32_t)np.side[0].pool.size();
  np.pool = np.side[0].pool;
  np.pool.insert(np.pool.end(), np.side[1].pool.begin(), np.side[1].pool.end());
  for (const Ref &r : refs) {
    const int32_t *h = &np.side[r.side].hdr[(size_t)r.idx * TILE_HDR_INTS];
    for (int i = 0; i < TILE_HDR_INTS; ++i) np.hdr.push_back(i == 5 ? h[i] + (r.side ? base1 : 0) : h[i]);
  }
  np.n_tiles = (int)refs.size();
  np.p_cap = std::max(np.side[0].p_cap, np.side[1].p_cap);
  np.q_cap = std::max(np.side[0].q_cap, np.side[1].q_cap);
  np.meta_cap = std::max(np.side[0].meta_cap, np.side[1].meta_cap);
  return np;
}

}
```

### gnn_uds_amd/csrc/uds_hip.hip

```cpp
#include <hip/hip_runtime.h>

#include <algorithm>
#include <cmath>
#include <cstdarg>
#include <cstdio>
#include <cstring>
#include <new>
#include <numeric>
#include <string>
#include <vector>

#include "../../include/uds_hip.h"
#include <cstdlib>

#include "kernels_dense.hpp"
#include "kernels_sparse.hpp"
#include "kernels_backward.hpp"
#include "kernels_fused.hpp"
#include "kernels_fused_ws.hpp"
#include "kernels_rowgemm.hpp"
#include "kernels_wgrad.hpp"
#include "kernels_conv_stream.hpp"
#include "kernels_fused128.hpp"
#include "kernels_gemm.hpp"
// ... 1211 lines not shown
    h.col.assign(c, c + rp[r]);
    return h;
  };
  uds_tile_plan *tp = new (std::nothrow) uds_tile_plan;
  if (!tp) return fail(UDS_ENOMEM, "uds_tile_plan_create: host allocation failed");
  tp->plan = uds::build_network_plan(mk(adj_rowptr, adj_col, n_node, n_node), mk(eadj_rowptr, eadj_col, n_edge, n_edge),
                                     mk(incn_rowptr, incn_col, n_node, n_edge), mk(ince_rowptr, ince_col, n_edge, n_node),
                                     t_node, t_link, p_limit, q_limit);
  *out = tp;
  return UDS_OK;
}

int uds_tile_plan_destroy(uds_tile_plan_t *tp) {
  delete tp;
  return UDS_OK;
}

int uds_tile_plan_sizes(const uds_tile_plan_t *tp, int64_t *n_tiles, int64_t *pool_len, int32_t *caps3) {
  UDS_REQUIRE(tp != nullptr, "uds_tile_plan_sizes: NULL plan");
  if (n_tiles) *n_tiles = tp->plan.n_tiles;
  if (pool_len) *pool_len = (int64_t)tp->plan.pool.size();
  if (caps3) {
    caps3[0] = tp->plan.p_cap;
    caps3[1] = tp->plan.q_cap;
    caps3[2] = tp->plan.meta_cap;
  }
  return UDS_OK;
}

int uds_tile_plan_copy(const uds_tile_plan_t *tp, int32_t *hdr_out, int32_t *pool_out) {
  UDS_REQUIRE(tp && hdr_out && pool_out, "uds_tile_plan_copy: NULL argument");
  std::memcpy(hdr_out, tp->plan.hdr.data(), sizeof(int32_t) * tp->plan.hdr.size());
  std::memcpy(pool_out, tp->plan.pool.data(), sizeof(int32_t) * tp->plan.pool.size());
  return UDS_OK;
}

int uds_tile_plan_blocks(const uds_tile_plan_t *tp, int32_t *blocks_out, int64_t *stride_out) {
  UDS_REQUIRE(tp != nullptr, "uds_tile_plan_blocks: NULL plan");
  const int cap = uds::ell_block_cap(tp->plan.hdr, tp->plan.pool, tp->plan.n_tiles);
  UDS_REQUIRE(cap >= 0, "uds_tile_plan_blocks: a tile has more than 255 primary / 256 secondary rows (byte-wide local indices)");
  if (stride_out) *stride_out = cap;
  if (!blocks_out) return UDS_OK;
  std::vector<int32_t> bl;
  uds::build_ell_blocks(tp->plan.hdr, tp->plan.pool, tp->plan.n_tiles, cap, bl);
  std::memcpy(blocks_out, bl.data(), sizeof(int32_t) * (size_t)cap * tp->plan.n_tiles);
  return UDS_OK;
}

int64_t uds_spatial_workspace_floats(const uds_network_t *net, int64_t S, int64_t h, int64_t d) {
  if (!net) return 0;
  const int64_t N = net->adj->n_rows, E = net->edge_adj->n_rows;
  return PACKED_WEIGHT_FLOATS + S * 2 * (N + E) * h + align4(S * N * (d + 2)) + align4(S * E * (d + 2));
}


int64_t uds_spatial_packed_bytes(void) { return PACKED_WEIGHT_FLOATS * 4; }

int uds_spatial_pack_weights(const uds_spatial_params_t *p, int64_t fx, int64_t fe, int64_t h, int64_t d, void *packed_out,
                             uds_stream_t stream) {
  UDS_REQUIRE(p && packed_out && p->xe_k && p->ex_k && p->gx_k && p->ge_k, "uds_spatial_pack_weights: NULL argument");
  const bool wide = h == uds::F128_H && d == uds::F128_D && fx == 128 && (fe == 128 || fe == 64);
  UDS_REQUIRE(wide || (h == uds::FUSED_H && d == uds::FUSED_D && (fx == 64 || fx == 96) && (fe == 64 || fe == 96)),
              "uds_spatial_pack_weights: the fused kernels take h=32, d=64, fx, fe in {64, 96} or h=64, d=128, fx=128, fe in {64, 128} (got h=%lld d=%lld "
              "fx=%lld fe=%lld)", (long long)h, (long long)d, (long long)fx, (long long)fe);
  UDS_REQUIRE(aligned16(packed_out), "uds_spatial_pack_weights: output must be 16-byte aligned");
  hipStream_t st = static_cast<hipStream_t>(stream);
  uint4 *wq = reinterpret_cast<uint4 *>(packed_out);
  hipError_t he;
  const int o_small = wide ? 2048 : 768, o_big = wide ? 6144 : 2048;
  if ((he = pack_weights(p->xe_k, (int)fe, (int)h, wq, st)) != hipSuccess ||
      (he = pack_weights(p->gx_k, (int)(fx + h), (int)d, wq + o_small, st)) != hipSuccess ||
      (he = pack_weights(p->ex_k, (int)fx, (int)h, wq + o_small + o_big, st)) != hipSuccess ||
      (he = pack_weights(p->ge_k, (int)(fe + h), (int)d, wq + 2 * o_small + o_big, st)) != hipSuccess)
    return fail(UDS_EHIP, "uds_spatial_pack_weights: launch -> %s", hipGetErrorString(he));
  if (!wide && fx == 64 && fe == 64) {
    const int total = (int)((fx + h) / 16) * (int)(d / 32) * 64;
    hipLaunchKernelGGL(uds::k_pack_weight_frags32, dim3((total + 255) / 256), dim3(256), 0, st, p->gx_k, (int)(fx + h), (int)d, wq + WS_BIG32_OFF);
    hipLaunchKernelGGL(uds::k_pack_weight_frags32, dim3((total + 255) / 256), dim3(256), 0, st, p->ge_k, (int)(fe + h), (int)d, wq + WS_BIG32_OFF + WS_BIG32_LEN);
    const int ts = (int)(fe / 16) * (int)(h / 32) * 64;
    hipLaunchKernelGGL(uds::k_pack_weight_frags32, dim3((ts + 255) / 256), dim3(256), 0, st, p->xe_k, (int)fe, (int)h, wq + WS_SMALL32_OFF);
    hipLaunchKernelGGL(uds::k_pack_weight_frags32, dim3((ts + 255) / 256), dim3(256), 0, st, p->ex_k, (int)fx, (int)h, wq + WS_SMALL32_OFF + WS_SMALL32_LEN);
    if ((he = hipGetLastError()) != hipSuccess) return fail(UDS_EHIP, "uds_spatial_pack_weights: launch -> %s", hipGetErrorString(he));
  }
  return UDS_OK;
}

int uds_spatial_layer_forward(const uds_network_t *net, const uds_spatial_params_t *p, const float *x, int64_t fx,
                              const float *e, int64_t fe, int64_t S, int64_t h, int64_t d, int act, int flags, float *ws,
                              float *out_x, float *out_e, uds_stream_t stream) {
  return uds_spatial_layer_forward_split(net, p, x, fx, nullptr, 0, e, fe, nullptr, 0, S, h, d, act, flags, ws, out_x, out_e, stream);
}

static int spatial_forward_impl(const uds_network_t *net, const uds_spatial_params_t *p, const float *x, int64_t fxa,
                                const float *xb, int64_t fxb, const float *e, int64_t fea, const float *eb, int64_t feb,
                                const float *rem_x, const float *rem_e, int64_t S, int64_t h, int64_t d, int act, int flags,
                                float *ws, float *out_x, float *out_e, uds_stream_t stream);

int uds_spatial_layer_forward_split(const uds_network_t *net, const uds_spatial_params_t *p, const float *x, int64_t fxa,
                                    const float *xb, int64_t fxb, const float *e, int64_t fea, const float *eb, int64_t feb,
                                    int64_t S, int64_t h, int64_t d, int act, int flags, float *ws, float *out_x, float *out_e,
                                    uds_stream_t stream) {
  return spatial_forward_impl(net, p, x, fxa, xb, fxb, e, fea, eb, feb, nullptr, nullptr, S, h, d, act, flags, ws, out_x, out_e, stream);
}

int uds_spatial_layer_forward_rem(const uds_network_t *net, const uds_spatial_params_t *p, const float *x, int64_t fx,
                                  const float *e, int64_t fe, const float *rem_x, const float *rem_e, int64_t S, int64_t h,
                                  int64_t d, int act, int flags, float *ws, float *out_x, float *out_e, uds_stream_t stream) {
  UDS_REQUIRE(rem_x && rem_e, "uds_spatial_layer_forward_rem: NULL remainder");
  UDS_REQUIRE(aligned16(rem_x) && aligned16(rem_e), "uds_spatial_layer_forward_rem: rem_x / rem_e must be 16-byte aligned");
  return spatial_forward_impl(net, p, x, fx, nullptr, 0, e, fe, nullptr, 0, rem_x, rem_e, S, h, d, act, flags | UDS_FLAG_REQUIRE_FUSED, ws,
                              out_x, out_e, stream);
}

static int spatial_forward_impl(const uds_network_t *net, const uds_spatial_params_t *p, const float *x, int64_t fxa,
                                const float *xb, int64_t fxb, const float *e, int64_t fea, const float *eb, int64_t feb,
                                const float *rem_x, const float *rem_e, int64_t S, int64_t h, int64_t d, int act, int flags,
                                float *ws, float *out_x, float *out_e, uds_stream_t stream) {
  UDS_REQUIRE(net && p && x && e && ws && out_x && out_e, "uds_spatial_layer_forward: NULL argument");
  UDS_REQUIRE((xb != nullptr) == (fxb > 0) && (eb != nullptr) == (feb > 0), "uds_spatial_layer_forward_split: xb/fxb or eb/feb disagree");
  UDS_REQUIRE((!xb || (fxa == 64 && fxb == 32)) && (!eb || (fea == 64 && feb == 32)),
              "uds_spatial_layer_forward_split: a split input must be 64 + 32 columns (got %lld+%lld, %lld+%lld)", (long long)fxa,
              (long long)fxb, (long long)fea, (long long)feb);
  UDS_REQUIRE(aligned16(xb) && aligned16(eb), "uds_spatial_layer_forward_split: xb/eb must be 16-byte aligned");
  const int64_t fx = fxa + fxb, fe = fea + feb;
  if (xb || eb) flags |= UDS_FLAG_REQUIRE_FUSED;
  UDS_REQUIRE(p->xe_k && p->ex_k && p->ne_n_val && p->ne_e_val && p->gx_k && p->gx_as && p->gx_an && p->ge_k &&
                  p->ge_as && p->ge_an,
              "uds_spatial_layer_forward: NULL parameter tensor");
  UDS_REQUIRE(h > 0 && h % 4 == 0 && d > 0 && d % 4 == 0, "uds_spatial_layer_forward: h=%lld d=%lld must be multiples of 4",
              (long long)h, (long long)d);
  UDS_REQUIRE(act >= UDS_ACT_LINEAR && act <= UDS_ACT_HARD_SIGMOID, "uds_spatial_layer_forward: unknown activation %d", act);
  UDS_REQUIRE(out_x != x && out_e != e, "uds_spatial_layer_forward: outputs must not alias inputs");
  UDS_REQUIRE(aligned16(x) && aligned16(e) && aligned16(ws) && aligned16(out_x) && aligned16(out_e),
              "uds_spatial_layer_forward: x/e/workspace/outputs must be 16-byte aligned");
  const int64_t N = net->adj->n_rows, E = net->edge_adj->n_rows;
  hipStream_t st = static_cast<hipStream_t>(stream);
  if (S == 0) return UDS_OK;

  if (h == uds::F128_H && d == uds::F128_D && fx == 128 && (fe == 128 || fe == 64) && !xb && !eb && !(flags & UDS_FLAG_EXACT_FP32) &&
      net->slot[slot_index(128, (int)fe)].ok && net->slot[slot_index((int)fe, 128)].ok) {
    UDS_REQUIRE(aligned16(p->xe_b) && aligned16(p->ex_b) && aligned16(p->gx_as) && aligned16(p->gx_an) && aligned16(p->gx_b) &&
                    aligned16(p->ge_as) && aligned16(p->ge_an) && aligned16(p->ge_b),
                "uds_spatial_layer_forward: bias / attention vectors must be 16-byte aligned");
    const uint4 *wq = reinterpret_cast<const uint4 *>(p->packed);
    if (!wq) {
      int rc = uds_spatial_pack_weights(p, fx, fe, h, d, ws, stream);
      if (rc != UDS_OK) return rc;
      wq = reinterpret_cast<const uint4 *>(ws);
    } else {
      UDS_REQUIRE(aligned16(wq), "uds_spatial_layer_forward: packed weights must be 16-byte aligned");
    }
    uds::FusedArgs a;
    a.blocks = nullptr;
    a.side[0] = uds::FusedSide{x, e, nullptr, nullptr, out_x, wq, wq + 2048, nullptr, nullptr, p->xe_b, p->gx_as, p->gx_an, p->gx_b, p->ne_n_val, (int)N, (int)E, rem_x};
    a.side[1] = uds::FusedSide{e, x, nullptr, nullptr, out_e, wq + 8192, wq + 10240, nullptr, nullptr, p->ex_b, p->ge_as, p->ge_an, p->ge_b, p->ne_e_val, (int)E, (int)N, rem_e};
    a.S = (int)S;
    a.act = act;
    a.dbg = nullptr;
#ifdef UDS_PHASE_TIMING
    a.dbg = reinterpret_cast<unsigned long long *>(ws + PACKED_WEIGHT_FLOATS);
#endif
    auto launch_side = [&](const uds_plan_slot &u, int side, auto FP_, auto FS_) {
      a.hdr = side < 0 ? u.d_hdr : u.d_hdr_side[side];
      a.pool = u.d_pool;
      a.n_tiles = side < 0 ? u.plan.n_tiles : u.plan.side[side].n_tiles;
      a.p_cap = u.plan.p_cap;
      a.q_cap = u.plan.q_cap;
      a.meta_cap = u.plan.meta_cap;
      a.side_mask = side < 0 ? 3 : (1 << side);
      if ((rem_x || rem_e) && a.p_cap > 64) return hipErrorInvalidValue;
      int64_t chunk = S, best = INT64_MAX;
      for (int64_t c = 1; c <= S; ++c) {
        const int64_t rounds = (((S + c - 1) / c) * a.n_tiles + 255) / 256;
        const int64_t cost = rounds * (3 + 2 * c);
        if (cost < best || (cost == best && c < chunk)) {
          best = cost;
          chunk = c;
        }
      }
      a.chunk = (int)chunk;
      const int grid = (int)(((S + chunk - 1) / chunk) * a.n_tiles);
      return launch_fused128<decltype(FP_)::value, decltype(FS_)::value>(a, grid, u.lds_bytes, st);
    };
    using I64 = std::integral_constant<int, 64>;
    using I128 = std::integral_constant<int, 128>;
    hipError_t he;
    if (fe == 128) {
      he = launch_side(net->slot[4], -1, I128{}, I128{});
    } else {
      he = launch_side(net->slot[5], 0, I128{}, I64{});
      if (he == hipSuccess) he = launch_side(net->slot[6], 1, I64{}, I128{});
    }
    if (he != hipSuccess) return fail(UDS_EHIP, "uds_spatial_layer_forward: fused d=128 launch -> %s", hipGetErrorString(he));
    return UDS_OK;
  }
  UDS_REQUIRE((!rem_x && !rem_e) || (h == uds::FUSED_H && d == uds::FUSED_D && fxa == 64 && fea == 64),
              "uds_spatial_layer_forward_rem: the remainder goes into the d = 128 fused kernel or the 64-wide d = 64 one (fx=%lld fe=%lld h=%lld d=%lld, plan %d)",
              (long long)fxa, (long long)fea, (long long)h, (long long)d, (int)(net->slot[4].ok));
  const bool shape_ok = h == uds::FUSED_H && d == uds::FUSED_D && (fx == 64 || fx == 96) && (fe == 64 || fe == 96) &&
                        std::max(N, E) * 384 < ((int64_t)1 << 31);
  const uds_plan_slot &sl = net->slot[slot_index((int)fx, (int)fe)];
  const uds_plan_slot &sl_link = net->slot[slot_index((int)fe, (int)fx)];
  if (flags & UDS_FLAG_REQUIRE_FUSED)
    UDS_REQUIRE(sl.ok && sl_link.ok && shape_ok && !(flags & UDS_FLAG_EXACT_FP32),
                "uds_spatial_layer_forward: fused kernel unavailable (plan %d, fx=%lld fe=%lld h=%lld d=%lld)", (int)sl.ok,
                (long long)fx, (long long)fe, (long long)h, (long long)d);
  if (sl.ok && sl_link.ok && shape_ok && !(flags & UDS_FLAG_EXACT_FP32)) {
    UDS_REQUIRE(aligned16(p->xe_b) && aligned16(p->ex_b) && aligned16(p->gx_as) && aligned16(p->gx_an) && aligned16(p->gx_b) &&
                    aligned16(p->ge_as) && aligned16(p->ge_an) && aligned16(p->ge_b),
                "uds_spatial_layer_forward: bias / attention vectors must be 16-byte aligned");
    hipError_t he;
    const uint4 *wq = reinterpret_cast<const uint4 *>(p->packed);
    if (!wq) {
      int rc = uds_spatial_pack_weights(p, fx, fe, h, d, ws, stream);
      if (rc != UDS_OK) return rc;
      wq = reinterpret_cast<const uint4 *>(ws);
    } else {
      UDS_REQUIRE(aligned16(wq), "uds_spatial_layer_forward: packed weights must be 16-byte aligned");
    }
    const uint4 *w_small_n = wq, *w_big_n = wq + 768, *w_small_e = wq + 768 + 2048, *w_big_e = wq + 2 * 768 + 2048;
    uds::FusedArgs a;
    a.blocks = nullptr;
    const bool has32 = fx == 64 && fe == 64;
    a.side[0] = uds::FusedSide{x, e, xb, eb, out_x, w_small_n, w_big_n, has32 ? wq + WS_BIG32_OFF : nullptr, has32 ? wq + WS_SMALL32_OFF : nullptr, p->xe_b, p->gx_as, p->gx_an, p->gx_b, p->ne_n_val, (int)N, (int)E, rem_x};
    a.side[1] = uds::FusedSide{e, x, eb, xb, out_e, w_small_e, w_big_e, has32 ? wq + WS_BIG32_OFF + WS_BIG32_LEN : nullptr, has32 ? wq + WS_SMALL32_OFF + WS_SMALL32_LEN : nullptr, p->ex_b, p->ge_as, p->ge_an, p->ge_b, p->ne_e_val, (int)E, (int)N, rem_e};
    int64_t lds_need = 0;
    auto use_plan = [&](const uds_plan_slot &u, int side) {
      a.hdr = side < 0 ? u.d_hdr : u.d_hdr_side[side];
      a.pool = u.d_pool;
      a.n_tiles = side < 0 ? u.plan.n_tiles : u.plan.side[side].n_tiles;
      a.p_cap = u.plan.p_cap;
      a.q_cap = u.plan.q_cap;
      a.meta_cap = u.blk_cap;
      a.blocks = side < 0 ? u.d_blocks : u.d_blocks_side[side];
      lds_need = u.lds_bytes;
    };
    use_plan(sl, -1);
    a.S = (int)S;
    a.act = act;
    a.dbg = nullptr;
#ifdef UDS_PHASE_TIMING
    a.dbg = reinterpret_cast<unsigned long long *>(ws + PACKED_WEIGHT_FLOATS);
#endif
    auto set_chunk = [&](int64_t working_tiles) {
      int64_t chunk = S, best = INT64_MAX;
      for (int64_t c = 1; c <= S; ++c) {
        const int64_t n_c = (S + c - 1) / c;
        const int64_t rounds = (n_c * working_tiles + 255) / 256;
        const int64_t cost = rounds * (3 + 2 * c);
        if (cost < best || (cost == best && c < chunk)) {
          best = cost;
          chunk = c;
        }
      }
#ifdef UDS_KNOBS
      if (const char *ov = std::getenv("UDS_CHUNK")) chunk = std::max<int64_t>(1, std::min<int64_t>(S, std::atoll(ov)));
#endif
      a.chunk = (int)chunk;
      return (int)(((S + chunk - 1) / chunk) * a.n_tiles);
    };
    if (fx == fe) {
      a.side_mask = 3;
      const int grid = set_chunk(a.n_tiles);
      const int64_t ws_lds = uds::fused_ws_lds_bytes(a.p_cap, a.q_cap, a.meta_cap);
      bool ws = fx == 64 && !xb && !eb && ws_lds <= FUSED_LDS_BUDGET && a.p_cap <= 128 && a.q_cap <= 256;
#ifdef UDS_NO_WS
      ws = false;
#endif
      UDS_REQUIRE(ws || (!rem_x && !rem_e), "uds_spatial_layer_forward_rem: the wave-specialised d = 64 kernel cannot take this network's plan (p_cap %d, q_cap %d, %lld B of LDS)",
                  a.p_cap, a.q_cap, (long long)ws_lds);
      if (ws) he = launch_fused_ws(a, grid, ws_lds, st);
      else he = (fx == 64) ? launch_fused<64, 64>(a, grid, lds_need, st) : launch_fused<96, 96>(a, grid, lds_need, st);
    } else {
      a.side_mask = 1;
      use_plan(sl, 0);
      int grid = set_chunk(a.n_tiles);
      he = (fx == 64) ? launch_fused<64, 96>(a, grid, lds_need, st) : launch_fused<96, 64>(a, grid, lds_need, st);
      if (he == hipSuccess) {
        a.side_mask = 2;
        use_plan(sl_link, 1);
        grid = set_chunk(a.n_tiles);
        he = (fe == 64) ? launch_fused<64, 96>(a, grid, lds_need, st) : launch_fused<96, 64>(a, grid, lds_need, st);
      }
    }
    if (he != hipSuccess) return fail(UDS_EHIP, "uds_spatial_layer_forward: fused launch -> %s", hipGetErrorString(he));
    return UDS_OK;
  }

  float *base = ws + PACKED_WEIGHT_FLOATS;
  float *x_e = base;
  float *e_x = x_e + S * E * h;
  float *agg_n = e_x + S * N * h;
  float *agg_e = agg_n + S * N * h;
  float *gat_ws_n = agg_e + S * E * h;
  float *gat_ws_e = gat_ws_n + align4(S * N * (d + 2));
  int rc;
  if ((rc = uds_dense_act(e, fe, nullptr, 0, S * E, p->xe_k, p->xe_b, h, act, nullptr, nullptr, x_e, nullptr, nullptr, stream))) return rc;
  if ((rc = uds_dense_act(x, fx, nullptr, 0, S * N, p->ex_k, p->ex_b, h, act, nullptr, nullptr, e_x, nullptr, nullptr, stream))) return rc;
  if ((rc = uds_csr_spmm(net->inc_n, p->ne_n_val, x_e, S, h, nullptr, UDS_ACT_LINEAR, agg_n, stream))) return rc;
  if ((rc = uds_csr_spmm(net->inc_e, p->ne_e_val, e_x, S, h, nullptr, UDS_ACT_LINEAR, agg_e, stream))) return rc;
  if ((rc = uds_gat_forward(net->adj, x, fx, agg_n, h, S, p->gx_k, p->gx_as, p->gx_an, p->gx_b, d, act, gat_ws_n, out_x, stream))) return rc;
  if ((rc = uds_gat_forward(net->edge_adj, e, fe, agg_e, h, S, p->ge_k, p->ge_as, p->ge_an, p->ge_b, d, act, gat_ws_e, out_e, stream))) return rc;
  return UDS_OK;
}

}
```

### gnn_uds_amd/layers.py

```python
import math
import os

import numpy as np
import torch
from torch import nn

from . import _lib
from . import autograd as _ag
from .graph import CSR, DrainageGraph, csr_from_dense


def _param(t):
    return nn.Parameter(t, requires_grad=False)


def _glorot_uniform(shape, device, generator=None):
    if len(shape) == 1:
        fan_in = fan_out = shape[0]
    elif len(shape) == 2:
        fan_in, fan_out = shape
    else:
        rf = int(np.prod(shape[:-2]))
        fan_in, fan_out = shape[-2] * rf, shape[-1] * rf
    limit = math.sqrt(6.0 / (fan_in + fan_out))
# ... 333 lines not shown
                or rest.shape[1] < 64:
            return None
        if self._rest_packed is None:
            self._rest_packed = _lib.remainder_pack(rest)
        return _lib.remainder_forward_dense(self._rest_packed, tuple(rest.shape), es.contiguous(), _packed_kernel(dense, dense.kernel), dense.bias,
                                            dense.activation, dense.units)

    def handle(self):
        if self._handle is None:
            self._handle = _lib.CsrHandle(self.csr)
        return self._handle

    def forward(self, x):
        if x.shape[-2] != self.shape[1]:
            raise _lib.UdsError('NodeEdge expects %d elements on axis -2, got %r' % (self.shape[1], tuple(x.shape)))
        xs, lead = _flatten_snapshots(x)
        if _ag.grad_on(xs, self.weight, self.bias):
            flat, ival = self._flat.to(self.weight.device), self._ival.to(self.weight.device)
            if self.sparse:
                val = self.weight * ival + self.bias
                out = _ag.SpmmFn.apply(val, xs, self.handle())
            else:
                val = self.weight.reshape(-1)[flat] * ival + self.bias.reshape(-1)[flat]
                out = _ag.SpmmFn.apply(val, xs, self.handle())
                if self.bias.requires_grad:
                    off = torch.ones_like(self.bias)
                    off.reshape(-1)[flat] = 0.0
                    rest = self.bias * off
                    if self.precision == 'bf16x3' and xs.shape[-1] % 4 == 0 and xs.shape[-1] <= 64:
                        out = out + _ag.RemainderFn.apply(rest, xs)
                    else:
                        out = out + torch.matmul(rest, xs)
            return out.reshape(lead + out.shape[-2:])
        val, rest = self.support_values()
        out = _lib.csr_spmm(self.handle(), val, xs)
        if rest is not None:
            out = out + self.remainder(xs, self.precision)
        return out.reshape(lead + out.shape[-2:])


class SpatialLayer(nn.Module):

    def __init__(self, graph, embed_size, activation='relu', fx=None, fe=None, sparse_params=None, net=None,
                 generator=None, precision='bf16x3', conv='GAT', filters=None):
        super().__init__()
        if conv not in ('GAT', 'GCN', 'Diffusion'):
            raise NotImplementedError('conv=%r: GAT, GCN and Diffusion are built' % (conv,))
        if conv != 'GAT' and filters is None:
            raise ValueError("conv=%r needs filters=(preprocess(adj), preprocess(edge_adj)) of its layer class" % (conv,))
        self.conv, self.filters = conv, filters
        if precision not in _lib.PRECISION_FLAGS:
            raise ValueError("precision must be 'bf16x3' (fused kernel, split-bf16 MFMA, fp32 accumulate) or 'fp32' "
                             "(exact-fp32 unfused kernels), got %r" % (precision,))
        self.precision = precision
        if not isinstance(graph, DrainageGraph):
            raise TypeError('graph must be a gnn_uds_amd.graph.DrainageGraph')
        self.graph, self.d, self.h, self.activation = graph, int(embed_size), int(embed_size) // 2, activation
        if self.d % 8:
            raise ValueError('embed_size must be a multiple of 8 (float4 rows of width d/2), got %d' % self.d)
        if sparse_params is None:
            sparse_params = graph.n_node * graph.n_edge > (1 << 24)
        fx = self.d if fx is None else int(fx)
        fe = self.d if fe is None else int(fe)
        g = generator
        self.dense_xe = Dense(self.h, activation, in_features=fe, generator=g, precision=precision)
        self.dense_ex = Dense(self.h, activation, in_features=fx, generator=g, precision=precision)
        abs_n = CSR(graph.inc_n.rowptr, graph.inc_n.col, graph.n_node, graph.n_edge, np.abs(graph.inc_n.val))
        abs_e = CSR(graph.inc_e.rowptr, graph.inc_e.col, graph.n_edge, graph.n_node, np.abs(graph.inc_e.val))
        self.node_edge_n = NodeEdge(abs_n, sparse=sparse_params, generator=g)
        self.node_edge_e = NodeEdge(abs_e, sparse=sparse_params, generator=g)
        self.node_edge_n.precision = self.node_edge_e.precision = precision
        if conv == 'GAT':
            self.gat_x = GATConv(self.d, activation=activation, in_channels=fx + self.h, generator=g)
            self.gat_e = GATConv(self.d, activation=activation, in_channels=fe + self.h, generator=g)
            self.gat_x.precision = self.gat_e.precision = precision
        elif conv == 'GCN':
            self.gcn_x = GCNConv(self.d, activation=activation, in_channels=fx + self.h, generator=g)
            self.gcn_e = GCNConv(self.d, activation=activation, in_channels=fe + self.h, generator=g)
        else:
            self.gcn_x = DiffusionConv(self.d, activation=activation, generator=g)
            self.gcn_e = DiffusionConv(self.d, activation=activation, generator=g)
        self._net = net
        self._packed = None
        self.last_path = None

    def _packed_weights(self, p, fx, fe, remainder=False):
        ks = (self.dense_xe.kernel, self.dense_ex.kernel, self.gat_x.kernel, self.gat_e.kernel)
        key = tuple((k._version, k.data_ptr()) for k in ks) + (fx, fe, remainder)
        if self._packed is None or self._packed[0] != key:
            if remainder:
                z = torch.zeros((self.h, self.h), device=p['xe_k'].device)
                aug = dict(xe_k=torch.cat([p['xe_k'], z]), ex_k=torch.cat([p['ex_k'], z]),
                           gx_k=torch.cat([p['gx_k'], p['gx_k'][-self.h:]]), ge_k=torch.cat([p['ge_k'], p['ge_k'][-self.h:]]))
                p = dict(p, **aug)
            else:
                aug = {}
            self._packed = (key, _lib.spatial_pack_weights(p, fx, fe, self.h, self.d), aug)
        return self._packed[1], self._packed[2]

    def _d128_remainder_ok(self, xs, es, xbs, ebs):
        if not (self.precision == 'bf16x3' and self.h == 64 and self.d == 128 and xs.shape[-1] == 128 and es.shape[-1] in (64, 128)
                and xbs is None and ebs is None):
            return False
        net = self.network()
        net.prepare(128, es.shape[-1])
        return bool(net.plan_info()['fused'] & (8 if es.shape[-1] == 128 else 16))

    def network(self):
        if self._net is None:
            self._net = _lib.NetworkHandle(self.graph)
        return self._net

    PACK_ROWS = 128

    def pack_factor(self):
        rows = max(self.graph.n_node, self.graph.n_edge)
        return max(1, self.PACK_ROWS // rows) if rows <= self.PACK_ROWS // 2 else 1

    def _replica(self, k):
        if getattr(self, '_rep', None) is None or self._rep[0] != k:
            self._rep = (k, _lib.NetworkHandle(self.graph.replicated(k)))
        return self._rep[1]

    def export_params(self):
        c = lambda t: None if t is None else t.detach().cpu().clone()
        if self.conv != 'GAT':
            raise NotImplementedError('export_params covers the GAT layer')
        p = dict(xe_k=c(self.dense_xe.kernel), xe_b=c(self.dense_xe.bias), ex_k=c(self.dense_ex.kernel),
                 ex_b=c(self.dense_ex.bias),
                 gx_k=c(self.gat_x.kernel), gx_as=c(self.gat_x.attn_kernel_self), gx_an=c(self.gat_x.attn_kernel_neighs),
                 gx_b=c(self.gat_x.bias),
                 ge_k=c(self.gat_e.kernel), ge_as=c(self.gat_e.attn_kernel_self), ge_an=c(self.gat_e.attn_kernel_neighs),
                 ge_b=c(self.gat_e.bias))
        for tag, ne in (('n', self.node_edge_n), ('e', self.node_edge_e)):
            if ne.sparse:
                p['ne_%s_v' % tag] = c(ne.support_values()[0])
            else:
                p['ne_%s_w' % tag], p['ne_%s_b' % tag] = c(ne.weight), c(ne.bias)
        return p

    def forward(self, x, e, xb=None, eb=None, adj_mask=None, attn_dropout=None):
        if adj_mask is not None:
            if self.conv != 'GAT':
                raise NotImplementedError('use_adj is built for conv=GAT (GCN / Diffusion would re-normalise the filter per snapshot)')
            if xb is not None:
                x = torch.cat([x, xb], dim=-1)
            if eb is not None:
                e = torch.cat([e, eb], dim=-1)
            xs, lead_x = _flatten_snapshots(x)
            es, lead_e = _flatten_snapshots(e)
            net = self.network()
            x_e, e_x = self.dense_xe(es), self.dense_ex(xs)
            ox = self.gat_x([xs, net.adj], xb=self.node_edge_n(x_e), edge_mask=adj_mask, attn_dropout=attn_dropout)
            oe = self.gat_e([es, net.edge_adj], xb=self.node_edge_e(e_x), attn_dropout=attn_dropout)
            self.last_path = 'unfused'
            return ox.reshape(lead_x + ox.shape[-2:]), oe.reshape(lead_e + oe.shape[-2:])
        fused_split = (xb is not None or eb is not None) and self.conv == 'GAT' and self.precision == 'bf16x3' and \
            self.h == 32 and self.d == 64 and x.shape[-1] + (0 if xb is None else xb.shape[-1]) in (64, 96) and \
            e.shape[-1] + (0 if eb is None else eb.shape[-1]) in (64, 96) and (xb is None or (x.shape[-1], xb.shape[-1]) == (64, 32)) and \
            (eb is None or (e.shape[-1], eb.shape[-1]) == (64, 32)) and not _ag.grad_on(x, e, xb, eb, *self.parameters()) and \
            self.node_edge_n.support_values()[1] is None and self.node_edge_e.support_values()[1] is None
        if not fused_split:
            if xb is not None:
                x = torch.cat([x, xb], dim=-1)
            if eb is not None:
                e = torch.cat([e, eb], dim=-1)
            xb = eb = None
        xs, lead_x = _flatten_snapshots(x)
        es, lead_e = _flatten_snapshots(e)
        xbs = None if xb is None else _flatten_snapshots(xb)[0]
        ebs = None if eb is None else _flatten_snapshots(eb)[0]
        if self.conv != 'GAT':
            x_e, e_x = self.dense_xe(es), self.dense_ex(xs)
            ox = self.gcn_x([torch.cat([xs, self.node_edge_n(x_e)], dim=-1), self.filters[0]])
            oe = self.gcn_e([torch.cat([es, self.node_edge_e(e_x)], dim=-1), self.filters[1]])
            return ox.reshape(lead_x + ox.shape[-2:]), oe.reshape(lead_e + oe.shape[-2:])
        if attn_dropout is not None or _ag.grad_on(xs, es, *self.parameters()):
            net = self.network()
            x_e, e_x = self.dense_xe(es), self.dense_ex(xs)
            ox = self.gat_x([xs, net.adj], xb=self.node_edge_n(x_e), attn_dropout=attn_dropout)
            oe = self.gat_e([es, net.edge_adj], xb=self.node_edge_e(e_x), attn_dropout=attn_dropout)
            return ox.reshape(lead_x + ox.shape[-2:]), oe.reshape(lead_e + oe.shape[-2:])
        vn, rest_n = self.node_edge_n.support_values()
        ve, rest_e = self.node_edge_e.support_values()
        p = dict(xe_k=self.dense_xe.kernel, xe_b=self.dense_xe.bias, ex_k=self.dense_ex.kernel, ex_b=self.dense_ex.bias,
                 ne_n_val=vn, ne_e_val=ve,
                 gx_k=self.gat_x.kernel, gx_as=self.gat_x.attn_kernel_self, gx_an=self.gat_x.attn_kernel_neighs,
                 gx_b=self.gat_x.bias,
                 ge_k=self.gat_e.kernel, ge_as=self.gat_e.attn_kernel_self, ge_an=self.gat_e.attn_kernel_neighs,
                 ge_b=self.gat_e.bias)
        self.last_path = 'unfused'
        if rest_n is not None or rest_e is not None:
            net = self.network()

            def remainders():
                S_, N_, E_ = xs.shape[0], xs.shape[1], es.shape[1]
                if rest_n is None:
                    rem_n = torch.zeros((S_, N_, self.h), device=xs.device, dtype=torch.float32)
                else:
                    rem_n = self.node_edge_n.remainder_of_dense(es, self.dense_xe) if not os.environ.get('UDS_REMAINDER_MATERIALISE') else None
                    if rem_n is None:
                        rem_n = self.node_edge_n.remainder(self.dense_xe(es))
                if rest_e is None:
                    rem_e = torch.zeros((S_, E_, self.h), device=xs.device, dtype=torch.float32)
                else:
                    rem_e = self.node_edge_e.remainder_of_dense(xs, self.dense_ex) if not os.environ.get('UDS_REMAINDER_MATERIALISE') else None
                    if rem_e is None:
                        rem_e = self.node_edge_e.remainder(self.dense_ex(xs))
                return rem_n, rem_e

            if self.precision == 'bf16x3' and self.h == 32 and self.d == 64 and xs.shape[-1] == 64 and es.shape[-1] == 64 \
                    and xbs is None and ebs is None:
                rem_n, rem_e = remainders()
                ox = None
                if getattr(self, '_ws_rem_ok', True):
                    try:
                        net.prepare(64, 64)
                        ox, oe = _lib.spatial_layer_forward(net, dict(p, packed=self._packed_weights(p, 64, 64)[0]), xs, es, self.h, self.d,
                                                            self.activation, _lib.PRECISION_FLAGS[self.precision], rem_x=rem_n, rem_e=rem_e)
                    except _lib.UdsError:
                        self._ws_rem_ok = False
                if ox is None:
                    packed, aug = self._packed_weights(p, 96, 96, remainder=True)
                    net.prepare(96, 96)
                    ox, oe = _lib.spatial_layer_forward(net, dict(p, packed=packed, **aug), xs, es, self.h, self.d, self.activation,
                                                        _lib.PRECISION_FLAGS[self.precision], xb=rem_n, eb=rem_e)
                self.last_path = 'fused+remainder'
            elif self._d128_remainder_ok(xs, es, xbs, ebs):
                rem_n, rem_e = remainders()
                packed = self._packed_weights(p, 128, es.shape[-1])[0]
                ox, oe = _lib.spatial_layer_forward(net, dict(p, packed=packed), xs, es, self.h, self.d, self.activation,
                                                    _lib.PRECISION_FLAGS[self.precision], rem_x=rem_n, rem_e=rem_e)
                self.last_path = 'fused+remainder'
            else:
                x_e, e_x = self.dense_xe(es), self.dense_ex(xs)
                ox = self.gat_x([xs, net.adj], xb=self.node_edge_n(x_e))
                oe = self.gat_e([es, net.edge_adj], xb=self.node_edge_e(e_x))
        else:
            fx = xs.shape[-1] + (0 if xbs is None else xbs.shape[-1])
            fe = es.shape[-1] + (0 if ebs is None else ebs.shape[-1])
            if self.precision == 'bf16x3' and self.h == 32 and self.d == 64 and fx in (64, 96) and fe in (64, 96):
                p['packed'] = self._packed_weights(p, fx, fe)[0]
                self.network().prepare(fx, fe)
            elif self.precision == 'bf16x3' and self.h == 64 and self.d == 128 and fx == 128 and fe in (64, 128) and xbs is None and ebs is None:
                self.network().prepare(128, fe)
                if self.network().plan_info()['fused'] & (8 if fe == 128 else 16):
                    p['packed'] = self._packed_weights(p, fx, fe)[0]
            if 'packed' not in p and self.precision == 'bf16x3' and fx % 32 == 0 and fe % 32 == 0 and self.h % 16 == 0 and self.d % 16 == 0 \
                    and xs.shape[0] * xs.shape[1] >= 4096:
                net = self.network()
                x_e, e_x = self.dense_xe(es), self.dense_ex(xs)
                ox = self.gat_x([xs, net.adj], xb=self.node_edge_n(x_e))
                oe = self.gat_e([es, net.edge_adj], xb=self.node_edge_e(e_x))
                return ox.reshape(lead_x + ox.shape[-2:]), oe.reshape(lead_e + oe.shape[-2:])
            k, S = self.pack_factor(), xs.shape[0]
            if 'packed' in p and k > 1 and S >= 16 * k:
                N, E, Sm = self.graph.n_node, self.graph.n_edge, S // k * k
                rep = self._replica(k)
                if self.d == 64:
                    rep.prepare(fx, fe)
                else:
                    rep.prepare(128, fe)
                pk = dict(p, ne_n_val=vn.repeat(k), ne_e_val=ve.repeat(k))
                v = lambda t, R: None if t is None else t[:Sm].reshape(Sm // k, k * R, t.shape[-1])
                ox, oe = _lib.spatial_layer_forward(rep, pk, v(xs, N), v(es, E), self.h, self.d, self.activation,
                                                    _lib.PRECISION_FLAGS[self.precision], xb=v(xbs, N), eb=v(ebs, E))
                ox, oe = ox.reshape(Sm, N, self.d), oe.reshape(Sm, E, self.d)
                if Sm < S:
                    t = lambda a: None if a is None else a[Sm:].contiguous()
                    rx, re = _lib.spatial_layer_forward(self.network(), p, t(xs), t(es), self.h, self.d, self.activation,
                                                        _lib.PRECISION_FLAGS[self.precision], xb=t(xbs), eb=t(ebs))
                    ox, oe = torch.cat([ox, rx]), torch.cat([oe, re])
                self.last_path = 'fused'
            else:
                ox, oe = _lib.spatial_layer_forward(self.network(), p, xs, es, self.h, self.d, self.activation,
                                                    _lib.PRECISION_FLAGS[self.precision], xb=xbs, eb=ebs)
                self.last_path = 'fused' if 'packed' in p else 'unfused'
        return ox.reshape(lead_x + ox.shape[-2:]), oe.reshape(lead_e + oe.shape[-2:])


class GraphBaseBlock(nn.Module):

    def __init__(self, n_node, n_edge, filt, embed_size, n_sp_layer, activation='relu', f_in=None, generator=None, conv='GAT',
                 precision='bf16x3'):
        super().__init__()
        if conv not in ('GAT', 'GCN', 'Diffusion'):
            raise NotImplementedError('conv=%r: GAT, GCN and Diffusion are built' % (conv,))
        self.n_node, self.n_edge, self.filt, self.conv = int(n_node), int(n_edge), filt, conv
        f_in = int(embed_size) if f_in is None else int(f_in)
        mk = {'GAT': GATConv, 'GCN': GCNConv, 'Diffusion': DiffusionConv}[conv]
        self.layers = nn.ModuleList([mk(embed_size, activation=activation, in_channels=(f_in if i == 0 else embed_size), generator=generator)
                                     for i in range(n_sp_layer)])
        for ly in self.layers:
            if conv == 'GAT':
                ly.precision = precision

    def forward(self, x, e, xb=None, eb=None, adj_mask=None, dropout=None, attn_dropout=None):
        if xb is not None:
            x = torch.cat([x, xb], dim=-1)
        if eb is not None:
            e = torch.cat([e, eb], dim=-1)
        if x.shape[-1] != e.shape[-1]:
            raise _lib.UdsError('graph_base stacks node and link rows: widths %d and %d differ' % (x.shape[-1], e.shape[-1]))
        if adj_mask is not None and self.conv != 'GAT':
            raise NotImplementedError('use_adj is built for conv=GAT')
        z = torch.cat([x, e], dim=-2)
        for ly in self.layers:
            if attn_dropout is not None and self.conv == 'GAT':
                z = ly([z, self.filt], edge_mask=adj_mask, attn_dropout=attn_dropout)
            else:
                z = ly([z, self.filt], edge_mask=adj_mask) if adj_mask is not None else ly([z, self.filt])
            if dropout is not None:
                z = dropout(z)
        return z[..., :self.n_node, :].contiguous(), z[..., self.n_node:, :].contiguous()


class Dropout(nn.Module):

    def __init__(self, rate, stream=None, generator=None):
        super().__init__()
        if not 0.0 <= rate < 1.0:
            raise ValueError('dropout rate %r outside [0, 1)' % (rate,))
        self.rate = float(rate)
        self.stream = stream if stream is not None else DropoutStream(generator=generator)

    def forward(self, x, training=False):
        if not training or self.rate == 0.0:
            return x
        x = x.contiguous()
        offset = self.stream.take(x.numel())
        return _ag.DropoutFn.apply(x, self.rate, self.stream.seed, offset)


class DropoutStream:

    def __init__(self, seed=None, generator=None):
        if seed is None:
            seed = int(torch.randint(0, 2 ** 62, (1,), generator=generator).item())
        self.seed, self.offset = int(seed), 0

    def take(self, n):
        o = self.offset
        self.offset += (int(n) + 3) // 4 * 4
        return o

    def reseed(self, seed):
        self.seed, self.offset = int(seed), 0


class SpatialBlock(nn.Module):

    def __init__(self, graph, embed_size, n_sp_layer, activation='relu', fx=None, fe=None, sparse_params=None,
                 generator=None, precision='bf16x3', conv='GAT', filters=None):
        super().__init__()
        layers = []
        for i in range(n_sp_layer):
            layers.append(SpatialLayer(graph, embed_size, activation, fx if i == 0 else None, fe if i == 0 else None,
# ... 33 lines not shown
```

### include/uds_hip.h

```cpp
#ifndef UDS_HIP_H
#define UDS_HIP_H

#include <stdint.h>

#ifdef __cplusplus
extern "C" {
#endif

#define UDS_ABI_VERSION 22

enum {
  UDS_OK = 0,
  UDS_EINVAL = -22,
  UDS_ENOMEM = -12,
  UDS_EHIP = -5,
  UDS_ENOSYS = -38
};

enum {
  UDS_ACT_LINEAR = 0,
  UDS_ACT_RELU = 1,
  UDS_ACT_TANH = 2,
  UDS_ACT_SIGMOID = 3,
  UDS_ACT_HARD_SIGMOID = 4
// ... 108 lines not shown
  const void *f_packed;
  const float *f_bias;
  int32_t n_a, act_a, n_hidden, act_h, act_f;
} uds_heads_t;
int uds_dense_cumsum_heads(const float *x, int64_t B, int64_t T, int64_t R, const void *packed, const float *bias,
                           const float *res, int act, const uds_heads_t *heads, float *out, uds_stream_t stream);

int uds_cumsum_act(const float *x, const float *res, int64_t B, int64_t T, int64_t R, int64_t F, int act,
                   float *out, uds_stream_t stream);

int uds_attn_sum_pool(const float *x, const float *k, int64_t B, int64_t R, int64_t F, float *out, uds_stream_t stream);

int uds_dropout(const float *x, int64_t n, float rate, uint64_t seed, uint64_t offset, float *out, uds_stream_t stream);

int uds_flow_balance(const uds_csr_t *inc_n, const float *sign, const float *flow, int64_t S,
                     const float *scale_in, const float *scale_out, float *q_in, float *q_out,
                     uds_stream_t stream);

int uds_roll_update(const uds_csr_t *inc_n, const float *sign, const float *span_e, const float *mini_e,
                    const float *scale_in, const float *scale_out, const float *y, int64_t cy, const float *ey,
                    int64_t ce, const float *b, int64_t B, int64_t so, int64_t T, int flood, float *x, float *ex,
                    float *preds, uds_stream_t stream);

int64_t uds_gat_workspace_floats(int64_t n, int64_t S, int64_t d);

int uds_gat_forward(const uds_csr_t *graph, const float *xa, int64_t fa, const float *xb,
                    int64_t fb, int64_t S, const float *W, const float *a_self,
                    const float *a_nbr, const float *bias, int64_t d, int act, float *workspace,
                    float *out, uds_stream_t stream);

int uds_gat_aggregate(const uds_csr_t *graph, const float *hx, const float *s_self, const float *s_nbr,
                      const float *bias, int64_t S, int64_t d, int act, float *out, uds_stream_t stream);


int uds_gat_aggregate_masked(const uds_csr_t *graph, const float *hx, const float *s_self, const float *s_nbr,
                             const float *bias, const float *edge_mask, int64_t S, int64_t d, int act, float *out,
                             uds_stream_t stream);

int uds_gat_backward(const uds_csr_t *graph, const uds_csr_t *graph_t, const int32_t *perm_t, const float *grad,
                     const float *hx, const float *s_self, const float *s_nbr, const float *a_self,
                     const float *a_nbr, int64_t S, int64_t d, float *alpha_ws, float *de_ws, float *d_hx,
                     float *ds_self, float *ds_nbr, uds_stream_t stream);

int uds_gat_aggregate_coef(const uds_csr_t *g, const float *hx, const float *s_self, const float *s_nbr, const float *bias,
                           const float *coef, int64_t S, int64_t d, int act, float *out, uds_stream_t stream);
int uds_gat_backward_coef(const uds_csr_t *g, const uds_csr_t *gt, const int32_t *perm_t, const float *grad, const float *hx,
                          const float *s_self, const float *s_nbr, const float *a_self, const float *a_nbr, const float *coef,
                          int64_t S, int64_t d, float *alpha_ws, float *de_ws, float *d_hx, float *ds_self, float *ds_nbr,
                          uds_stream_t stream);

int uds_gat_aggregate_ex(const uds_csr_t *g, const float *hx, const float *s_self, const float *s_nbr, const float *bias,
                         const float *edge_mask, const float *coef, int64_t S, int64_t d, int act, float *out,
                         uds_stream_t stream);
int uds_gat_backward_ex(const uds_csr_t *g, const uds_csr_t *gt, const int32_t *perm_t, const float *grad, const float *hx,
                        const float *s_self, const float *s_nbr, const float *a_self, const float *a_nbr,
                        const float *edge_mask, const float *coef, int64_t S, int64_t d, float *alpha_ws, float *de_ws,
                        float *d_hx, float *ds_self, float *ds_nbr, uds_stream_t stream);

int uds_csr_sddmm(const uds_csr_t *csr, const float *a, const float *b, int64_t S, int64_t F, float *out,
                  uds_stream_t stream);

int64_t uds_wgrad_workspace_floats(int64_t rows, int64_t F, int64_t H, int with_bias);
int uds_wgrad(const float *a, const float *g, int64_t B, int64_t T, int64_t R, int64_t F, int64_t H, int64_t shift,
              int with_bias, float *workspace, float *d_kernel, float *d_bias, uds_stream_t stream);

typedef struct uds_network uds_network_t;

int uds_network_create(const uds_csr_t *adj, const uds_csr_t *edge_adj, const uds_csr_t *inc_n,
                       const uds_csr_t *inc_e, uds_network_t **out);
int uds_network_destroy(uds_network_t *net);
int uds_network_prepare(uds_network_t *net, int64_t fx, int64_t fe);
int uds_network_plan_info(const uds_network_t *net, int32_t *info8);

typedef struct uds_tile_plan uds_tile_plan_t;
int uds_tile_plan_create(const int32_t *adj_rowptr, const int32_t *adj_col, const int32_t *eadj_rowptr,
                         const int32_t *eadj_col, const int32_t *incn_rowptr, const int32_t *incn_col,
                         const int32_t *ince_rowptr, const int32_t *ince_col, int64_t n_node,
                         int64_t n_edge, int32_t t_node, int32_t t_link, int32_t p_limit,
                         int32_t q_limit, uds_tile_plan_t **out);
int uds_tile_plan_destroy(uds_tile_plan_t *plan);
int uds_tile_plan_sizes(const uds_tile_plan_t *plan, int64_t *n_tiles, int64_t *pool_len, int32_t *caps3);
int uds_tile_plan_copy(const uds_tile_plan_t *plan, int32_t *hdr_out, int32_t *pool_out);
int uds_tile_plan_blocks(const uds_tile_plan_t *plan, int32_t *blocks_out, int64_t *stride_out);

typedef struct uds_spatial_params {
  const float *xe_k, *xe_b;
  const float *ex_k, *ex_b;
  const float *ne_n_val;
  const float *ne_e_val;
  const float *gx_k, *gx_as, *gx_an, *gx_b;
  const float *ge_k, *ge_as, *ge_an, *ge_b;
  const void *packed;
} uds_spatial_params_t;

int64_t uds_spatial_packed_bytes(void);
int uds_spatial_pack_weights(const uds_spatial_params_t *params, int64_t fx, int64_t fe, int64_t h, int64_t d,
                             void *packed_out, uds_stream_t stream);

enum {
  UDS_FLAG_EXACT_FP32 = 1,
  UDS_FLAG_REQUIRE_FUSED = 2
};

int64_t uds_spatial_workspace_floats(const uds_network_t *net, int64_t S, int64_t h, int64_t d);

int uds_spatial_layer_forward(const uds_network_t *net, const uds_spatial_params_t *params,
                              const float *x, int64_t fx, const float *e, int64_t fe, int64_t S,
                              int64_t h, int64_t d, int act, int flags, float *workspace,
                              float *out_x, float *out_e, uds_stream_t stream);

int uds_spatial_layer_forward_split(const uds_network_t *net, const uds_spatial_params_t *params, const float *xa,
                                    int64_t fxa, const float *xb, int64_t fxb, const float *ea, int64_t fea,
                                    const float *eb, int64_t feb, int64_t S, int64_t h, int64_t d, int act, int flags,
                                    float *workspace, float *out_x, float *out_e, uds_stream_t stream);

int uds_spatial_layer_forward_rem(const uds_network_t *net, const uds_spatial_params_t *params, const float *x, int64_t fx,
                                  const float *e, int64_t fe, const float *rem_x, const float *rem_e, int64_t S, int64_t h,
                                  int64_t d, int act, int flags, float *workspace, float *out_x, float *out_e,
                                  uds_stream_t stream);

#ifdef __cplusplus
}
#endif
#endif
```

Baseline: 289,600.

## Pre-resolve node-edge incidence values into cached ELL tile blocks

Adds a pass that bakes the node-edge incidence values (ne_n_val/ne_e_val) into a copy of each ELL tile block, so the fused kernels no longer gather those values through global indices and skip one block-wide barrier. The resolved image is cached per layer, keyed on the identity of the value tensors and the network, and passed through a new params field. The warp-specialised kernel also gets an optional early-load path that prefetches the tile metadata and attention vectors into registers before staging them. The cost is extra memory for the resolved image and the risk of stale values if the incidence tensors are modified in place.

```diff
diff --git a/gnn_uds_amd/_lib.py b/gnn_uds_amd/_lib.py
--- a/gnn_uds_amd/_lib.py
+++ b/gnn_uds_amd/_lib.py
@@ -96,10 +96,13 @@
     'uds_tile_plan_sizes': (_c_int, [_c_ptr, ctypes.POINTER(_c_i64), ctypes.POINTER(_c_i64), _c_ptr]),
     'uds_tile_plan_copy': (_c_int, [_c_ptr, _c_ptr, _c_ptr]),
     'uds_tile_plan_blocks': (_c_int, [_c_ptr, _c_ptr, ctypes.POINTER(_c_i64)]),
+    'uds_tile_plan_resolve': (_c_int, [_c_ptr, _c_ptr, _c_ptr, _c_ptr]),
     'uds_roll_update': (_c_int, [_c_ptr] * 7 + [_c_i64, _c_ptr, _c_i64, _c_ptr, _c_i64, _c_i64, _c_i64, _c_int, _c_ptr, _c_ptr, _c_ptr, _c_ptr]),
     'uds_spatial_workspace_floats': (_c_i64, [_c_ptr, _c_i64, _c_i64, _c_i64]),
     'uds_spatial_packed_bytes': (_c_i64, []),
     'uds_spatial_pack_weights': (_c_int, [_c_ptr, _c_i64, _c_i64, _c_i64, _c_i64, _c_ptr, _c_ptr]),
+    'uds_spatial_node_edge_bytes': (_c_i64, [_c_ptr, _c_i64, _c_i64]),
+    'uds_spatial_pack_node_edge': (_c_int, [_c_ptr, _c_ptr, _c_i64, _c_i64, _c_ptr, _c_ptr]),
     'uds_spatial_layer_forward': (_c_int, [_c_ptr, _c_ptr, _c_ptr, _c_i64, _c_ptr, _c_i64, _c_i64, _c_i64, _c_i64, _c_int,
                                            _c_int, _c_ptr, _c_ptr, _c_ptr, _c_ptr]),
     'uds_spatial_layer_forward_rem': (_c_int, [_c_ptr, _c_ptr, _c_ptr, _c_i64, _c_ptr, _c_i64, _c_ptr, _c_ptr, _c_i64, _c_i64, _c_i64, _c_int, _c_int,
@@ -111,7 +114,7 @@
 
 class SpatialParams(ctypes.Structure):
     _fields_ = [(n, _c_ptr) for n in ('xe_k', 'xe_b', 'ex_k', 'ex_b', 'ne_n_val', 'ne_e_val',
-                                      'gx_k', 'gx_as', 'gx_an', 'gx_b', 'ge_k', 'ge_as', 'ge_an', 'ge_b', 'packed')]
+                                      'gx_k', 'gx_as', 'gx_an', 'gx_b', 'ge_k', 'ge_as', 'ge_an', 'ge_b', 'packed', 'ne_resolved')]
 
 
 class UdsError(RuntimeError):
@@ -294,7 +297,7 @@
             _lib.uds_network_destroy(h)
 
 
-def tile_plan(graph, t_node=48, t_link=48, p_limit=0, q_limit=0, blocks=False):
+def tile_plan(graph, t_node=48, t_link=48, p_limit=0, q_limit=0, blocks=False, resolve=None):
     lib = load()
     arrs = []
     for c in (graph.adj, graph.edge_adj, graph.inc_n, graph.inc_e):
@@ -309,17 +312,26 @@
         hdr = np.zeros((nt.value, 8), dtype=np.int32)
         pool = np.zeros(pl.value, dtype=np.int32)
         _check(lib.uds_tile_plan_copy(h, hdr.ctypes.data, pool.ctypes.data), 'uds_tile_plan_copy')
-        blk = None
+        blk = res = None
         if blocks:
             stride = _c_i64()
             if lib.uds_tile_plan_blocks(h, None, ctypes.byref(stride)) == 0:
                 blk = np.zeros((nt.value, stride.value), dtype=np.int32)
                 _check(lib.uds_tile_plan_blocks(h, blk.ctypes.data, ctypes.byref(stride)), 'uds_tile_plan_blocks')
+                if resolve is not None:
+                    vn, ve = (np.ascontiguousarray(v, dtype=np.float32) for v in resolve)
+                    if vn.size != graph.inc_n.nnz or ve.size != graph.inc_e.nnz:
+                        raise UdsError('tile_plan: resolve takes one value per incidence entry (%d, %d), got %d, %d' %
+                                       (graph.inc_n.nnz, graph.inc_e.nnz, vn.size, ve.size))
+                    res = np.zeros_like(blk)
+                    _check(lib.uds_tile_plan_resolve(h, vn.ctypes.data, ve.ctypes.data, res.ctypes.data), 'uds_tile_plan_resolve')
     finally:
         lib.uds_tile_plan_destroy(h)
     out = dict(p_cap=int(caps[0]), q_cap=int(caps[1]), meta_cap=int(caps[2]))
     if blocks:
         out['blocks'] = blk
+        if resolve is not None:
+            out['resolved'] = res
     return hdr, pool, out
 
 
@@ -1004,9 +1016,9 @@
 def _spatial_params(p):
     sp = SpatialParams()
     for name, _ in SpatialParams._fields_:
-        if name == 'packed':
-            t = p.get('packed')
-            sp.packed = None if t is None else t.data_ptr()
+        if name in ('packed', 'ne_resolved'):
+            t = p.get(name)
+            setattr(sp, name, None if t is None else t.data_ptr())
         else:
             setattr(sp, name, _dev(p[name], name, allow_none=name.endswith('_b')))
     return sp
@@ -1019,6 +1031,19 @@
     q['packed'] = None
     _check(lib.uds_spatial_pack_weights(ctypes.byref(_spatial_params(q)), fx, fe, h, d, out.data_ptr(), _stream()),
            'uds_spatial_pack_weights')
+    return out
+
+
+def spatial_pack_node_edge(net, p, fx, fe):
+    lib = load()
+    net.prepare(fx, fe)
+    n = lib.uds_spatial_node_edge_bytes(net.ptr, fx, fe)
+    if n <= 0:
+        return None
+    out = torch.empty(n // 4, device=p['ne_n_val'].device, dtype=torch.int32)
+    sp = SpatialParams()
+    sp.ne_n_val, sp.ne_e_val = _dev(p['ne_n_val'], 'ne_n_val'), _dev(p['ne_e_val'], 'ne_e_val')
+    _check(lib.uds_spatial_pack_node_edge(net.ptr, ctypes.byref(sp), fx, fe, out.data_ptr(), _stream()), 'uds_spatial_pack_node_edge')
     return out
 
 
diff --git a/gnn_uds_amd/csrc/kernels_fused.hpp b/gnn_uds_amd/csrc/kernels_fused.hpp
--- a/gnn_uds_amd/csrc/kernels_fused.hpp
+++ b/gnn_uds_amd/csrc/kernels_fused.hpp
@@ -28,7 +28,15 @@
   const float *b_small, *a_self, *a_nbr, *b_out, *ne_val;
   int n_prim_glob, n_sec_glob;
   const float *rem;
+  const int32_t *ne_res;
 };
+
+__global__ void k_resolve_blocks(const int32_t *__restrict__ blocks, int stride, const float *__restrict__ val0,
+                                 const float *__restrict__ val1, int32_t *__restrict__ out) {
+  const int32_t *b = blocks + (int64_t)blockIdx.x * stride;
+  const float *val = b[6] ? val1 : val0;
+  for (int i = threadIdx.x; i < stride; i += blockDim.x) out[(int64_t)blockIdx.x * stride + i] = ell_resolved_word(b, i, val);
+}
 
 struct FusedArgs {
   FusedSide side[2];
@@ -340,8 +348,9 @@
     for (int i = tid; i < N_COLD_S; i += NT) cold_s[i] = S_.w_small[T_COLD_S * MB_S * 2 * 64 + i];
   f32x4 bo = f32x4{0.f, 0.f, 0.f, 0.f};
   if (S_.b_out) bo = *reinterpret_cast<const f32x4 *>(S_.b_out + 4 * c16);
+  const bool resolved = S_.ne_res != nullptr;
   {
-    const uint4 *src = reinterpret_cast<const uint4 *>(a.blocks + (int64_t)tile * a.meta_cap);
+    const uint4 *src = reinterpret_cast<const uint4 *>((resolved ? S_.ne_res : a.blocks) + (int64_t)tile * a.meta_cap);
     uint4 *dst = reinterpret_cast<uint4 *>(smem);
     for (int i = tid; i < a.meta_cap / 4; i += NT) dst[i] = src[i];
   }
@@ -435,17 +444,19 @@
 #ifdef UDS_PHASE_TIMING
   const unsigned long long t_dma_issued_ = clock64();
 #endif
-  for (int i = tid; i < ELL_INC * n_prim; i += NT) {
-    const int k = inc_w[i];
-    reinterpret_cast<float *>(inc_w)[i] = k >= 0 ? S_.ne_val[k] : 0.f;
-  }
-  if (flags & ELL_FLAG_INC_OVF)
-    for (int i = tid; i < n_ovf; i += NT) reinterpret_cast<float *>(ovf_w)[i] = S_.ne_val[ovf_w[i]];
+  if (!resolved) {
+    for (int i = tid; i < ELL_INC * n_prim; i += NT) {
+      const int k = inc_w[i];
+      reinterpret_cast<float *>(inc_w)[i] = k >= 0 ? S_.ne_val[k] : 0.f;
+    }
+    if (flags & ELL_FLAG_INC_OVF)
+      for (int i = tid; i < n_ovf; i += NT) reinterpret_cast<float *>(ovf_w)[i] = S_.ne_val[ovf_w[i]];
+  }
   const float *ovf_val = reinterpret_cast<const float *>(ovf_w);
 #ifdef UDS_PHASE_TIMING
   const unsigned long long t_loads_issued_ = clock64();
 #endif
-  __syncthreads();
+  if (!resolved) __syncthreads();
   UDS_STAMP(0);
 
   auto phase1 = [&](int s) {
diff --git a/gnn_uds_amd/csrc/kernels_fused_ws.hpp b/gnn_uds_amd/csrc/kernels_fused_ws.hpp
--- a/gnn_uds_amd/csrc/kernels_fused_ws.hpp
+++ b/gnn_uds_amd/csrc/kernels_fused_ws.hpp
@@ -112,8 +112,30 @@
   float *hx = sec + 2 * a.q_cap * SEC_STRIDE;
   const int sec_buf = a.q_cap * SEC_STRIDE, hx_buf = a.p_cap * FUSED_D;
 
+#ifdef UDS_PHASE_TIMING
+  unsigned long long tm_[8] = {0, 0, 0, 0, 0, 0, 0, 0}, tl_ = clock64();
+  const unsigned long long rt0_ = __builtin_amdgcn_s_memrealtime(), mt0_ = tl_;
+#define WS_STAMP(k) do { const unsigned long long n_ = clock64(); tm_[k] += n_ - tl_; tl_ = n_; } while (0)
+#define WS_DUMP() do { if (a.dbg && lane == 0) { unsigned long long *o = a.dbg + ((size_t)blockIdx.x * 8 + wave) * 16; \
+    for (int q_ = 0; q_ < 7; ++q_) o[q_] = tm_[q_]; o[12] = wave; \
+    o[15] = ((__builtin_amdgcn_s_memrealtime() - rt0_) << 32) | ((clock64() - mt0_) & 0xffffffffull); \
+    o[7] = 1ull | ((unsigned long long)sd << 8) | ((unsigned long long)n_own << 16) | ((unsigned long long)n_prim << 32) | ((unsigned long long)n_sec << 48); } } while (0)
+#else
+#define WS_STAMP(k) do { } while (0)
+#define WS_DUMP() do { } while (0)
+#endif
+#ifdef UDS_WS_RESOLVED
+  const bool resolved = S_.ne_res != nullptr;
+#else
+  constexpr bool resolved = false;
+#define UDS_WS_PLAIN_COPY 1
+#endif
+#ifdef UDS_WS_PLAIN_COPY
+#ifndef UDS_WS_LATE_WSMALL
+#define UDS_WS_LATE_WSMALL 1
+#endif
   {
-    const uint4 *src = reinterpret_cast<const uint4 *>(a.blocks + (int64_t)tile * a.meta_cap);
+    const uint4 *src = reinterpret_cast<const uint4 *>((resolved ? S_.ne_res : a.blocks) + (int64_t)tile * a.meta_cap);
     uint4 *dst = reinterpret_cast<uint4 *>(smem);
     for (int i = tid; i < a.meta_cap / 4; i += NT) dst[i] = src[i];
   }
@@ -123,6 +145,42 @@
     if (tid < FUSED_H) attn[2 * FUSED_D + tid] = S_.b_small ? S_.b_small[tid] : 0.f;
     attn[2 * FUSED_D + FUSED_H + tid] = S_.b_out ? S_.b_out[tid] : 0.f;
   }
+#else
+  const uint4 *blk_src = reinterpret_cast<const uint4 *>((resolved ? S_.ne_res : a.blocks) + (int64_t)tile * a.meta_cap);
+  const int blk_n4 = a.meta_cap / 4;
+  uint4 blk0 = make_uint4(0u, 0u, 0u, 0u);
+  if (tid < blk_n4) blk0 = blk_src[tid];
+  float v_as = 0.f, v_an = 0.f, v_bs = 0.f, v_bo = 0.f;
+  if (tid < FUSED_D) {
+    v_as = S_.a_self[tid];
+    v_an = S_.a_nbr[tid];
+    if (tid < FUSED_H && S_.b_small) v_bs = S_.b_small[tid];
+    if (S_.b_out) v_bo = S_.b_out[tid];
+  }
+  auto stash = [&]() __attribute__((always_inline)) {
+    uint4 *dst = reinterpret_cast<uint4 *>(smem);
+    if (tid < blk_n4) dst[tid] = blk0;
+    for (int i = tid + NT; i < blk_n4; i += NT) dst[i] = blk_src[i];
+    if (tid < FUSED_D) {
+      attn[tid] = v_as * 1.44269504088896340736f;
+      attn[FUSED_D + tid] = v_an * 1.44269504088896340736f;
+      if (tid < FUSED_H) attn[2 * FUSED_D + tid] = v_bs;
+      attn[2 * FUSED_D + FUSED_H + tid] = v_bo;
+    }
+  };
+#if !defined(UDS_WS_MFMA16) && !defined(UDS_WS_LATE_WSMALL)
+  bf16x8 wq[8];
+  if (team_y) {
+    stash();
+  } else {
+#pragma unroll
+    for (int i = 0; i < 8; ++i) wq[i] = __builtin_bit_cast(bf16x8, S_.w_small32[i * 64 + lane]);
+    stash();
+  }
+#else
+  stash();
+#endif
+#endif
   __syncthreads();
   const int n_own = __builtin_amdgcn_readfirstlane(smem[0]), n_prim = __builtin_amdgcn_readfirstlane(smem[1]),
             n_sec = __builtin_amdgcn_readfirstlane(smem[2]), flags = __builtin_amdgcn_readfirstlane(smem[3]),
@@ -139,30 +197,24 @@
   int32_t *ovf_w = smem + off.ovf_w;
   const int32_t *adj_ptr = smem + off.adj_ptr, *adj_loc = smem + off.adj_loc;
 
-  for (int i = tid; i < ELL_INC * n_prim; i += NT) {
-    const int k = inc_w[i];
-    reinterpret_cast<float *>(inc_w)[i] = k >= 0 ? S_.ne_val[k] : 0.f;
+  if (!resolved) {
+    for (int i = tid; i < ELL_INC * n_prim; i += NT) {
+      const int k = inc_w[i];
+      reinterpret_cast<float *>(inc_w)[i] = k >= 0 ? S_.ne_val[k] : 0.f;
+    }
+    if (flags & ELL_FLAG_INC_OVF)
+      for (int i = tid; i < n_ovf; i += NT) reinterpret_cast<float *>(ovf_w)[i] = S_.ne_val[ovf_w[i]];
   }
-  if (flags & ELL_FLAG_INC_OVF)
-    for (int i = tid; i < n_ovf; i += NT) reinterpret_cast<float *>(ovf_w)[i] = S_.ne_val[ovf_w[i]];
   const float *ovf_val = reinterpret_cast<const float *>(ovf_w);
 
-#ifdef UDS_PHASE_TIMING
-  unsigned long long tm_[8] = {0, 0, 0, 0, 0, 0, 0, 0}, tl_ = clock64();
-  const unsigned long long rt0_ = __builtin_amdgcn_s_memrealtime(), mt0_ = tl_;
-#define WS_STAMP(k) do { const unsigned long long n_ = clock64(); tm_[k] += n_ - tl_; tl_ = n_; } while (0)
-#define WS_DUMP() do { if (a.dbg && lane == 0) { unsigned long long *o = a.dbg + ((size_t)blockIdx.x * 8 + wave) * 16; \
-    for (int q_ = 0; q_ < 7; ++q_) o[q_] = tm_[q_]; o[12] = wave; \
-    o[15] = ((__builtin_amdgcn_s_memrealtime() - rt0_) << 32) | ((clock64() - mt0_) & 0xffffffffull); \
-    o[7] = 1ull | ((unsigned long long)sd << 8) | ((unsigned long long)n_own << 16) | ((unsigned long long)n_prim << 32) | ((unsigned long long)n_sec << 48); } } while (0)
-#else
-#define WS_STAMP(k) do { } while (0)
-#define WS_DUMP() do { } while (0)
-#endif
   const int64_t sec_stride = (int64_t)S_.n_sec_glob * FS, prim_stride = (int64_t)S_.n_prim_glob * FP;
   const int n_snap = s_end - s_begin;
 
+#ifdef UDS_WS_KEEP_BAR2
   __syncthreads();
+#else
+  if (!resolved) __syncthreads();
+#endif
   if (team_y) {
 #ifndef UDS_WS_MFMA16
     typedef float f32x16 __attribute__((ext_vector_type(16)));
@@ -542,11 +594,17 @@
     typedef float f32x16 __attribute__((ext_vector_type(16)));
     constexpr int KS32 = FS / 16, SJ32 = (8 + NX - 1) / NX;
     const int n32 = lane & 31, hf = lane >> 5;
+    static_assert(KS32 * 2 == 8, "the fragments requested at the top of the kernel");
     bf16x8 w1h[KS32], w1l[KS32];
 #pragma unroll
     for (int t = 0; t < KS32; ++t) {
+#ifndef UDS_WS_LATE_WSMALL
+      w1h[t] = wq[t * 2 + 0];
+      w1l[t] = wq[t * 2 + 1];
+#else
       w1h[t] = __builtin_bit_cast(bf16x8, S_.w_small32[(t * 2 + 0) * 64 + lane]);
       w1l[t] = __builtin_bit_cast(bf16x8, S_.w_small32[(t * 2 + 1) * 64 + lane]);
+#endif
     }
     unsigned srow[SJ32];
 #pragma unroll
diff --git a/gnn_uds_amd/csrc/tile_plan.hpp b/gnn_uds_amd/csrc/tile_plan.hpp
--- a/gnn_uds_amd/csrc/tile_plan.hpp
+++ b/gnn_uds_amd/csrc/tile_plan.hpp
@@ -431,6 +431,25 @@
   }
 }
 
+UDS_HD inline int32_t ell_resolved_word(const int32_t *block, int i, const float *val) {
+  const int n_own = block[0], n_prim = block[1], n_sec = block[2], flags = block[3], n_ovf = block[4], n_adj = block[5];
+  const EllOffsets o = ell_offsets(n_own, n_prim, n_sec, flags, n_ovf, n_adj);
+  const int32_t k = block[i];
+  float v;
+  if (i >= o.inc_w && i < o.inc_w + ELL_INC * n_prim) v = k >= 0 ? val[k] : 0.f;
+  else if ((flags & ELL_FLAG_INC_OVF) && i >= o.ovf_w && i < o.ovf_w + n_ovf) v = val[k];
+  else return k;
+  int32_t r;
+  __builtin_memcpy(&r, &v, sizeof r);
+  return r;
+}
+inline void resolve_ell_blocks(const int32_t *blocks, int n_tiles, int stride, const float *const val[2], int32_t *out) {
+  for (int t = 0; t < n_tiles; ++t) {
+    const int32_t *b = blocks + (size_t)stride * t;
+    for (int i = 0; i < stride; ++i) out[(size_t)stride * t + i] = ell_resolved_word(b, i, val[b[6]]);
+  }
+}
+
 inline int64_t fused_lds_bytes(int p_cap, int q_cap, int meta_cap, int h, int d, int fp, int fs) {
   const int64_t weights = 16 * 64 * 2 * ((int64_t)(fs / 32) * (h / 16) + (int64_t)((fp + h) / 32) * (d / 16));
   const int64_t stage = std::max<int64_t>(4 * ((int64_t)q_cap * fs + (int64_t)p_cap * fp), weights);
diff --git a/gnn_uds_amd/csrc/uds_hip.hip b/gnn_uds_amd/csrc/uds_hip.hip
--- a/gnn_uds_amd/csrc/uds_hip.hip
+++ b/gnn_uds_amd/csrc/uds_hip.hip
@@ -1317,6 +1317,68 @@
     hipLaunchKernelGGL(uds::k_pack_weight_frags32, dim3((ts + 255) / 256), dim3(256), 0, st, p->ex_k, (int)fx, (int)h, wq + WS_SMALL32_OFF + WS_SMALL32_LEN);
     if ((he = hipGetLastError()) != hipSuccess) return fail(UDS_EHIP, "uds_spatial_pack_weights: launch -> %s", hipGetErrorString(he));
   }
+  return UDS_OK;
+}
+
+struct ne_image_list {
+  const int32_t *d_blocks;
+  int n_tiles, stride;
+  int64_t off_ints;
+};
+static bool ne_image_lists(const uds_network_t *net, int64_t fx, int64_t fe, ne_image_list (&ls)[2], int &n_lists, int64_t &total_ints) {
+  n_lists = 0;
+  total_ints = 0;
+  if (!net || !((fx == 64 || fx == 96) && (fe == 64 || fe == 96))) return false;
+  const uds_plan_slot &sl = net->slot[slot_index((int)fx, (int)fe)];
+  const uds_plan_slot &sl_link = net->slot[slot_index((int)fe, (int)fx)];
+  if (!sl.ok || !sl_link.ok) return false;
+  if (fx == fe) {
+    ls[n_lists++] = ne_image_list{sl.d_blocks, sl.plan.n_tiles, sl.blk_cap, 0};
+  } else {
+    ls[n_lists++] = ne_image_list{sl.d_blocks_side[0], sl.plan.side[0].n_tiles, sl.blk_cap, 0};
+    ls[n_lists++] = ne_image_list{sl_link.d_blocks_side[1], sl_link.plan.side[1].n_tiles, sl_link.blk_cap, (int64_t)sl.plan.side[0].n_tiles * sl.blk_cap};
+  }
+  total_ints = ls[n_lists - 1].off_ints + (int64_t)ls[n_lists - 1].n_tiles * ls[n_lists - 1].stride;
+  return true;
+}
+
+int64_t uds_spatial_node_edge_bytes(const uds_network_t *net, int64_t fx, int64_t fe) {
+  ne_image_list ls[2];
+  int n_lists;
+  int64_t total;
+  if (!ne_image_lists(net, fx, fe, ls, n_lists, total)) return 0;
+  return 4 * std::max<int64_t>(total, 4);
+}
+
+int uds_spatial_pack_node_edge(const uds_network_t *net, const uds_spatial_params_t *p, int64_t fx, int64_t fe, void *out,
+                               uds_stream_t stream) {
+  UDS_REQUIRE(net && p && out && p->ne_n_val && p->ne_e_val, "uds_spatial_pack_node_edge: NULL argument");
+  UDS_REQUIRE(aligned16(out), "uds_spatial_pack_node_edge: output must be 16-byte aligned");
+  ne_image_list ls[2];
+  int n_lists;
+  int64_t total;
+  UDS_REQUIRE(ne_image_lists(net, fx, fe, ls, n_lists, total),
+              "uds_spatial_pack_node_edge: no fused d = 64 tile plan for fx=%lld fe=%lld (uds_network_prepare first; fx, fe in {64, 96})",
+              (long long)fx, (long long)fe);
+  hipStream_t st = static_cast<hipStream_t>(stream);
+  for (int i = 0; i < n_lists; ++i) {
+    if (ls[i].n_tiles == 0) continue;
+    hipLaunchKernelGGL(uds::k_resolve_blocks, dim3((unsigned)ls[i].n_tiles), dim3(256), 0, st, ls[i].d_blocks, ls[i].stride, p->ne_n_val,
+                       p->ne_e_val, reinterpret_cast<int32_t *>(out) + ls[i].off_ints);
+    hipError_t he = hipGetLastError();
+    if (he != hipSuccess) return fail(UDS_EHIP, "uds_spatial_pack_node_edge: launch -> %s", hipGetErrorString(he));
+  }
+  return UDS_OK;
+}
+
+int uds_tile_plan_resolve(const uds_tile_plan_t *tp, const float *val_node, const float *val_link, int32_t *resolved_out) {
+  UDS_REQUIRE(tp && val_node && val_link && resolved_out, "uds_tile_plan_resolve: NULL argument");
+  const int cap = uds::ell_block_cap(tp->plan.hdr, tp->plan.pool, tp->plan.n_tiles);
+  UDS_REQUIRE(cap >= 0, "uds_tile_plan_resolve: a tile has more than 255 primary / 256 secondary rows (byte-wide local indices)");
+  std::vector<int32_t> bl;
+  uds::build_ell_blocks(tp->plan.hdr, tp->plan.pool, tp->plan.n_tiles, cap, bl);
+  const float *const val[2] = {val_node, val_link};
+  uds::resolve_ell_blocks(bl.data(), tp->plan.n_tiles, cap, val, resolved_out);
   return UDS_OK;
 }
 
@@ -1459,6 +1521,8 @@
     const bool has32 = fx == 64 && fe == 64;
     a.side[0] = uds::FusedSide{x, e, xb, eb, out_x, w_small_n, w_big_n, has32 ? wq + WS_BIG32_OFF : nullptr, has32 ? wq + WS_SMALL32_OFF : nullptr, p->xe_b, p->gx_as, p->gx_an, p->gx_b, p->ne_n_val, (int)N, (int)E, rem_x};
     a.side[1] = uds::FusedSide{e, x, eb, xb, out_e, w_small_e, w_big_e, has32 ? wq + WS_BIG32_OFF + WS_BIG32_LEN : nullptr, has32 ? wq + WS_SMALL32_OFF + WS_SMALL32_LEN : nullptr, p->ex_b, p->ge_as, p->ge_an, p->ge_b, p->ne_e_val, (int)E, (int)N, rem_e};
+    const int32_t *ne_res = reinterpret_cast<const int32_t *>(p->ne_resolved);
+    UDS_REQUIRE(aligned16(ne_res), "uds_spatial_layer_forward: ne_resolved must be 16-byte aligned");
     int64_t lds_need = 0;
     auto use_plan = [&](const uds_plan_slot &u, int side) {
       a.hdr = side < 0 ? u.d_hdr : u.d_hdr_side[side];
@@ -1468,6 +1532,8 @@
       a.q_cap = u.plan.q_cap;
       a.meta_cap = u.blk_cap;
       a.blocks = side < 0 ? u.d_blocks : u.d_blocks_side[side];
+      a.side[0].ne_res = side == 1 ? nullptr : ne_res;
+      a.side[1].ne_res = !ne_res ? nullptr : side == 1 ? ne_res + (int64_t)sl.plan.side[0].n_tiles * sl.blk_cap : side < 0 ? ne_res : nullptr;
       lds_need = u.lds_bytes;
     };
     use_plan(sl, -1);
diff --git a/gnn_uds_amd/layers.py b/gnn_uds_amd/layers.py
--- a/gnn_uds_amd/layers.py
+++ b/gnn_uds_amd/layers.py
@@ -439,6 +439,8 @@
             self.gcn_e = DiffusionConv(self.d, activation=activation, generator=g)
         self._net = net
         self._packed = None
+        self._resolved = {}
+        self._resolved_flag = [False]
         self.last_path = None
 
     def _packed_weights(self, p, fx, fe, remainder=False):
@@ -454,6 +456,26 @@
                 aug = {}
             self._packed = (key, _lib.spatial_pack_weights(p, fx, fe, self.h, self.d), aug)
         return self._packed[1], self._packed[2]
+
+    resolve_blocks = True
+
+    @property
+    def last_resolved(self):
+        return self._resolved_flag[0]
+
+    def _resolved_blocks(self, net, vn, ve, fx, fe, copies=1):
+        flag = self._resolved_flag
+        flag[0] = False
+        if not self.resolve_blocks:
+            return None
+        hit = self._resolved.get((fx, fe, copies))
+        if hit is None or hit[0] is not vn or hit[1] is not ve or hit[2] is not net:
+            if vn.is_cuda and torch.cuda.is_current_stream_capturing():
+                return None
+            q = dict(ne_n_val=vn if copies == 1 else vn.repeat(copies), ne_e_val=ve if copies == 1 else ve.repeat(copies))
+            hit = self._resolved[(fx, fe, copies)] = (vn, ve, net, _lib.spatial_pack_node_edge(net, q, fx, fe))
+        flag[0] = hit[3] is not None
+        return hit[3]
 
     def _d128_remainder_ok(self, xs, es, xbs, ebs):
         if not (self.precision == 'bf16x3' and self.h == 64 and self.d == 128 and xs.shape[-1] == 128 and es.shape[-1] in (64, 128)
@@ -573,15 +595,16 @@
                 if getattr(self, '_ws_rem_ok', True):
                     try:
                         net.prepare(64, 64)
-                        ox, oe = _lib.spatial_layer_forward(net, dict(p, packed=self._packed_weights(p, 64, 64)[0]), xs, es, self.h, self.d,
+                        ox, oe = _lib.spatial_layer_forward(net, dict(p, packed=self._packed_weights(p, 64, 64)[0],
+                                                                      ne_resolved=self._resolved_blocks(net, vn, ve, 64, 64)), xs, es, self.h, self.d,
                                                             self.activation, _lib.PRECISION_FLAGS[self.precision], rem_x=rem_n, rem_e=rem_e)
                     except _lib.UdsError:
                         self._ws_rem_ok = False
                 if ox is None:
                     packed, aug = self._packed_weights(p, 96, 96, remainder=True)
                     net.prepare(96, 96)
-                    ox, oe = _lib.spatial_layer_forward(net, dict(p, packed=packed, **aug), xs, es, self.h, self.d, self.activation,
-                                                        _lib.PRECISION_FLAGS[self.precision], xb=rem_n, eb=rem_e)
+                    ox, oe = _lib.spatial_layer_forward(net, dict(p, packed=packed, ne_resolved=self._resolved_blocks(net, vn, ve, 96, 96), **aug),
+                                                        xs, es, self.h, self.d, self.activation, _lib.PRECISION_FLAGS[self.precision], xb=rem_n, eb=rem_e)
                 self.last_path = 'fused+remainder'
             elif self._d128_remainder_ok(xs, es, xbs, ebs):
                 rem_n, rem_e = remainders()
@@ -596,9 +619,11 @@
         else:
             fx = xs.shape[-1] + (0 if xbs is None else xbs.shape[-1])
             fe = es.shape[-1] + (0 if ebs is None else ebs.shape[-1])
+            fused64 = False
             if self.precision == 'bf16x3' and self.h == 32 and self.d == 64 and fx in (64, 96) and fe in (64, 96):
                 p['packed'] = self._packed_weights(p, fx, fe)[0]
                 self.network().prepare(fx, fe)
+                fused64 = True
             elif self.precision == 'bf16x3' and self.h == 64 and self.d == 128 and fx == 128 and fe in (64, 128) and xbs is None and ebs is None:
                 self.network().prepare(128, fe)
                 if self.network().plan_info()['fused'] & (8 if fe == 128 else 16):
@@ -619,17 +644,23 @@
                 else:
                     rep.prepare(128, fe)
                 pk = dict(p, ne_n_val=vn.repeat(k), ne_e_val=ve.repeat(k))
+                if fused64:
+                    pk['ne_resolved'] = self._resolved_blocks(rep, vn, ve, fx, fe, copies=k)
                 v = lambda t, R: None if t is None else t[:Sm].reshape(Sm // k, k * R, t.shape[-1])
                 ox, oe = _lib.spatial_layer_forward(rep, pk, v(xs, N), v(es, E), self.h, self.d, self.activation,
                                                     _lib.PRECISION_FLAGS[self.precision], xb=v(xbs, N), eb=v(ebs, E))
                 ox, oe = ox.reshape(Sm, N, self.d), oe.reshape(Sm, E, self.d)
                 if Sm < S:
                     t = lambda a: None if a is None else a[Sm:].contiguous()
+                    if fused64:
+                        p['ne_resolved'] = self._resolved_blocks(self.network(), vn, ve, fx, fe)
                     rx, re = _lib.spatial_layer_forward(self.network(), p, t(xs), t(es), self.h, self.d, self.activation,
                                                         _lib.PRECISION_FLAGS[self.precision], xb=t(xbs), eb=t(ebs))
                     ox, oe = torch.cat([ox, rx]), torch.cat([oe, re])
                 self.last_path = 'fused'
             else:
+                if fused64:
+                    p['ne_resolved'] = self._resolved_blocks(self.network(), vn, ve, fx, fe)
                 ox, oe = _lib.spatial_layer_forward(self.network(), p, xs, es, self.h, self.d, self.activation,
                                                     _lib.PRECISION_FLAGS[self.precision], xb=xbs, eb=ebs)
                 self.last_path = 'fused' if 'packed' in p else 'unfused'
diff --git a/include/uds_hip.h b/include/uds_hip.h
--- a/include/uds_hip.h
+++ b/include/uds_hip.h
@@ -214,6 +214,7 @@
 int uds_tile_plan_sizes(const uds_tile_plan_t *plan, int64_t *n_tiles, int64_t *pool_len, int32_t *caps3);
 int uds_tile_plan_copy(const uds_tile_plan_t *plan, int32_t *hdr_out, int32_t *pool_out);
 int uds_tile_plan_blocks(const uds_tile_plan_t *plan, int32_t *blocks_out, int64_t *stride_out);
+int uds_tile_plan_resolve(const uds_tile_plan_t *plan, const float *val_node, const float *val_link, int32_t *resolved_out);
 
 typedef struct uds_spatial_params {
   const float *xe_k, *xe_b;
@@ -223,11 +224,16 @@
   const float *gx_k, *gx_as, *gx_an, *gx_b;
   const float *ge_k, *ge_as, *ge_an, *ge_b;
   const void *packed;
+  const void *ne_resolved;
 } uds_spatial_params_t;
 
 int64_t uds_spatial_packed_bytes(void);
 int uds_spatial_pack_weights(const uds_spatial_params_t *params, int64_t fx, int64_t fe, int64_t h, int64_t d,
                              void *packed_out, uds_stream_t stream);
+
+int64_t uds_spatial_node_edge_bytes(const uds_network_t *net, int64_t fx, int64_t fe);
+int uds_spatial_pack_node_edge(const uds_network_t *net, const uds_spatial_params_t *params, int64_t fx, int64_t fe, void *out,
+                               uds_stream_t stream);
 
 enum {
   UDS_FLAG_EXACT_FP32 = 1,
```

Result: no change. 289,400 (median of 2 runs) (-0.1%).
